# zzz5y/street_crafter

Hardware: AMD Instinct MI355X
Metric: frames/sec @1M Gaussians 1920x1280 + PSNR vs ref; 1/2/4/8 MI355X (higher is better)
Workload: dtype f32

## Files before the change

### include/street_crafter_amd.h

```cpp
#ifndef STREET_CRAFTER_AMD_H
#define STREET_CRAFTER_AMD_H

#include <stddef.h>
#include <stdint.h>

#ifdef __cplusplus
extern "C" {
#endif

typedef void* sc_stream_t;

#define SC_OK 0
#define SC_EINVAL (-1)
#define SC_EWORKSPACE (-2)
#define SC_EUNSUPPORTED (-3)

const char* sc_version(void);
const char* sc_error_string(int code);
const char* sc_target_arch(void);
int sc_wait_i64(const int64_t* addr, int64_t value, int64_t timeout_us);

int sc_projection_fwd(const float* means, const float* quats, const float* scales,
                      const float* viewmats, const float* Ks, int C, int N, int width, int height,
                      float eps2d, float near_plane, float far_plane, float radius_clip,
// ... 2 lines not shown

int sc_projection_bwd(const float* means, const float* quats, const float* scales,
                      const float* viewmats, const float* Ks, int C, int N, int width, int height,
                      float eps2d, const int32_t* radii, const float* conics,
                      const float* compensations ,
                      const float* v_means2d, const float* v_depths, const float* v_conics,
                      const float* v_compensations ,
                      float* v_means, float* v_quats, float* v_scales, sc_stream_t stream);

size_t sc_isect_workspace_bytes(int64_t CN);
int sc_isect_count(const float* means2d, const int32_t* radii, int C, int N,
                   int tile_size, int tile_width, int tile_height,
                   int32_t* tiles_per_gauss, int64_t* total_dev, void* workspace, size_t ws_bytes,
                   sc_stream_t stream);
int sc_isect_emit(const float* means2d, const int32_t* radii, const float* depths, int C, int N,
                  int tile_size, int tile_width, int tile_height,
                  const int32_t* tiles_per_gauss, int64_t n_isects,
                  int64_t* isect_ids, int32_t* flatten_ids, void* workspace, size_t ws_bytes,
                  sc_stream_t stream);

size_t sc_radix_sort_workspace_bytes(int64_t n);
int sc_radix_sort_pairs_u64_i32(uint64_t* keys, int32_t* vals, uint64_t* tmp_keys, int32_t* tmp_vals,
                                int64_t n, int end_bit, void* workspace, size_t ws_bytes,
                                sc_stream_t stream);

size_t sc_isect_bin_workspace_bytes(int64_t CN, int C, int tile_width, int tile_height, int64_t n_records);
int sc_isect_bin_count(const float* means2d, const int32_t* radii, const float* depths, int C, int N,
                       int tile_size, int tile_width, int tile_height,
                       int32_t* tiles_per_gauss, int32_t* isect_offsets, int64_t* meta_dev ,
                       int64_t* meta_mirror , int64_t seq,
                       void* workspace, size_t ws_bytes,
                       const int32_t* tile_work ,
                       const float* viewmats ,
                       int32_t* view_registry ,
                       int32_t* tile_order ,
                       sc_stream_t stream);
int sc_view_slots(void);
int sc_view_registry_words(void);
int sc_isect_bin_bucket_capacity(void);
int sc_isect_split_limits(int64_t* out );
int64_t sc_isect_split_seg_bound(int64_t n_records, int nsb);
int sc_isect_split_bins(const uint64_t* keys, int64_t n, uint64_t lo, uint64_t hi, int32_t* bins);
int sc_isect_split_plan(const uint32_t* bin_counts, int cap, int32_t* range_of_bin, int32_t* n_ranges);
int sc_isect_bin_sort(const float* means2d, const int32_t* radii, const float* depths, int C, int N,
                      int tile_size, int tile_width, int tile_height,
                      const int32_t* isect_offsets, const int64_t* meta_dev,
                      void* count_workspace ,
                      int64_t capacity, int64_t rec_capacity, int64_t super_capacity,
                      int64_t* isect_ids , int32_t* flatten_ids,
                      void* workspace, size_t ws_bytes, sc_stream_t stream);
int sc_isect_ids_rebuild(const int32_t* flatten_ids, const int32_t* isect_offsets, const float* depths,
                         int C, int N, int tile_width, int tile_height, int64_t n_isects,
                         int64_t* isect_ids, sc_stream_t stream);
int sc_isect_bin_reset_cursors(void* count_workspace, int64_t CN, int C, int tile_width, int tile_height,
                               sc_stream_t stream);

int sc_isect_offsets(const int64_t* isect_ids, int64_t n_isects, int C, int tile_width,
                     int tile_height, int32_t* offsets, sc_stream_t stream);

int sc_sh_fwd(int degree, const float* dirs, const float* coeffs, const uint8_t* masks,
              int64_t M, int K, float* colors, sc_stream_t stream);
int sc_sh_bwd(int degree, const float* dirs, const float* coeffs, const uint8_t* masks,
              int64_t M, int K, const float* v_colors, float* v_coeffs, float* v_dirs,
              sc_stream_t stream);

int sc_rasterize_fwd(const float* means2d, const float* conics, const float* colors,
                     const float* opacities, const float* backgrounds, const uint8_t* tile_masks,
                     int C, int N, int D, int width, int height, int tile_size,
                     int tile_width, int tile_height,
                     const int32_t* isect_offsets, const int32_t* flatten_ids, int64_t n_isects,
                     float* render_colors, float* render_alphas,
                     int32_t* last_ids ,
                     const int32_t* tile_order ,
                     int32_t* tile_work ,
                     sc_stream_t stream);
int sc_tile_order_len(int total_tiles);
int sc_rasterize_bwd(const float* means2d, const float* conics, const float* colors,
                     const float* opacities, const float* backgrounds, const uint8_t* tile_masks,
                     int C, int N, int D, int width, int height, int tile_size,
                     int tile_width, int tile_height,
                     const int32_t* isect_offsets, const int32_t* flatten_ids, int64_t n_isects,
                     const float* render_alphas, const int32_t* last_ids,
                     const float* v_render_colors, const float* v_render_alphas,
                     float* v_means2d_abs, float* v_means2d, float* v_conics, float* v_colors,
                     float* v_opacities, const int32_t* tile_order ,
                     sc_stream_t stream);

size_t sc_knn_workspace_bytes(int64_t n);
int sc_knn3_mean_dist2(const float* points, int64_t n, float* out, void* workspace,
                       size_t ws_bytes, sc_stream_t stream);

int sc_point_project(const float* points, const float* colors, const float* opacities , float occ,
                     const float* radius_in , int N, const double* viewmat, double fx,
                     double fy, double cx, double cy, double focal_r, int width, int height, double near_plane,
                     double far_plane, int radius_mode, double scale, float knn_scale_down, int32_t* radii,
                     float* means2d, float* depths, float* records, sc_stream_t stream);
int sc_point_rasterize_fwd(const float* records, int N, int width, int height, int tile_width, int tile_height,
                           const int32_t* isect_offsets, const int32_t* flatten_ids, int64_t n_isects, int max_hit,
                           const float* background , float* out_rgb, int64_t pix_stride,
                           int64_t ch_stride, float* out_alpha, int64_t alpha_stride,
                           float* out_depth , sc_stream_t stream);

size_t sc_loss_workspace_bytes(int batch, int channels, int height, int width);
int sc_loss_fwd(const float* img1, const float* img2, const uint8_t* mask , const int64_t* strides_host,
                int batch, int channels, int height, int width, int mask_batch, int mask_height, int mask_width,
                int window, float* ssim_out, float* l1_out, int64_t* kept_out ,
// ... 80 lines not shown
} sc_densify_job;
typedef struct {
    const float* src_param;
    const float* src_exp_avg;
    const float* src_exp_avg_sq;
    float* dst_param;
    float* dst_exp_avg;
    float* dst_exp_avg_sq;
    const float* child;
    const int32_t* src_row;
    const uint8_t* slot;
    int64_t n, n_out;
    int32_t width;
    int32_t reserved;
} sc_densify_group;
int sc_densify_scan_block(void);
int sc_densify_max_jobs(void);
int sc_densify_max_groups(void);
size_t sc_densify_plan_workspace_bytes(const sc_densify_job* jobs_host, int n_jobs);
int sc_densify_plan(const sc_densify_job* jobs_host, int n_jobs, void* workspace, size_t workspace_bytes,
                    sc_stream_t stream);
int sc_densify_apply(const sc_densify_group* groups_host, int n_groups, sc_stream_t stream);

int sc_camera_centers(const float* viewmats, int C, float* out, sc_stream_t stream);
int sc_projection_sh_fwd(const float* means, const float* quats, const float* scales,
                         const float* opacities, const float* sh_coeffs, const float* viewmats,
                         const float* Ks, const float* camera_centers, int C, int N, int K,
                         int sh_degree, int width, int height, float eps2d, float near_plane,
                         float far_plane, float radius_clip, int antialiased, int32_t* radii,
                         float* means2d, float* depths, float* conics, float* opacities_out,
                         float* colors4,
                         float* records ,
                         sc_stream_t stream);
int sc_projection_sh_bwd(const float* means, const float* quats, const float* scales,
                         const float* opacities, const float* sh_coeffs, const float* viewmats,
                         const float* Ks, const float* camera_centers, int C, int N, int K,
                         int sh_degree, int width, int height, float eps2d, int antialiased,
                         const int32_t* radii, const float* conics, const float* v_means2d,
                         const float* v_depths, const float* v_conics, const float* v_opacities_out,
                         const float* v_colors4, float* v_means, float* v_quats, float* v_scales,
                         float* v_opacities, float* v_sh, sc_stream_t stream);
int sc_rasterize_fwd_packed(const float* records, const float* backgrounds, const uint8_t* tile_masks,
                            int C, int N, int width, int height, int tile_width, int tile_height,
                            const int32_t* isect_offsets, const int32_t* flatten_ids, int64_t n_isects,
                            float* render_colors, float* render_alphas, const int32_t* tile_order,
                            int32_t* tile_work, int depth_normalise, sc_stream_t stream);
int sc_rasterize_fwd_planar(const float* means2d, const float* conics, const float* colors,
                            const float* opacities, const float* backgrounds, const uint8_t* tile_masks,
                            int C, int N, int D, int width, int height, int tile_size,
                            int tile_width, int tile_height,
                            const int32_t* isect_offsets, const int32_t* flatten_ids, int64_t n_isects,
                            float* render_colors, float* render_alphas,
                            const int32_t* tile_order, int32_t* tile_work, sc_stream_t stream);
int sc_records_unpack(const float* records, int64_t CN, float* conics, float* opacities, float* colors4,
                      sc_stream_t stream);
int sc_rasterize_fwd_ed(const float* means2d, const float* conics, const float* colors,
                        const float* opacities, const float* backgrounds, const uint8_t* tile_masks,
                        int C, int N, int D, int width, int height, int tile_size, int tile_width,
                        int tile_height, const int32_t* isect_offsets, const int32_t* flatten_ids,
                        int64_t n_isects, float* render_colors, float* render_alphas,
                        const int32_t* tile_order, int32_t* tile_work, sc_stream_t stream);

int sc_group_extents(const int32_t* isect_offsets, const int32_t* flatten_ids, int64_t n_isects,
                     const uint8_t* group_ids , int C, int N, int n_groups,
                     int tile_width, int tile_height, int32_t* group_end, sc_stream_t stream);
int sc_rasterize_fwd_groups(const float* means2d, const float* conics, const float* colors,
                            const float* opacities, const uint8_t* group_ids, const int32_t* group_end,
                            int C, int N, int D, int n_groups, int width, int height, int tile_size,
                            int tile_width, int tile_height,
                            const int32_t* isect_offsets, const int32_t* flatten_ids, int64_t n_isects,
                            float* render_colors, float* render_alphas,
                            float* group_colors, float* group_alphas, sc_stream_t stream);

int sc_rasterize_fwd_groups_ids(const float* means2d, const float* conics, const float* colors,
                                const float* opacities, const uint8_t* group_ids, const int32_t* group_end,
                                int C, int N, int D, int n_groups, int width, int height, int tile_size,
                                int tile_width, int tile_height,
                                const int32_t* isect_offsets, const int32_t* flatten_ids, int64_t n_isects,
                                float* render_colors, float* render_alphas,
                                float* group_colors, float* group_alphas, int32_t* last_pos, sc_stream_t stream);
int sc_rasterize_bwd_groups(const float* means2d, const float* conics, const float* colors,
                            const float* opacities, const uint8_t* group_ids, int C, int N, int D, int n_groups,
                            int width, int height, int tile_size, int tile_width, int tile_height,
                            const int32_t* isect_offsets, const int32_t* flatten_ids, int64_t n_isects,
                            const float* render_alphas, const float* group_alphas, const int32_t* last_pos,
                            const float* v_render_colors, const float* v_render_alphas,
                            const float* v_group_colors, const float* v_group_alphas,
                            float* v_means2d_abs, float* v_means2d, float* v_conics, float* v_colors,
                            float* v_opacities, sc_stream_t stream);

int sc_rasterize_fwd_layers(const float* means2d, const float* conics, const float* colors,
                            const float* opacities, int C, int N, int D, int n_front, int width, int height,
                            int tile_size, int tile_width, int tile_height,
                            const int32_t* isect_offsets, const int32_t* flatten_ids, int64_t n_isects,
                            int epilogue, int rounding, float* out0, float* out1, float* out2, float* out3,
                            uint8_t* out_u8, int32_t* layer_begin, sc_stream_t stream);

int sc_frame_composite_u8(const float* fg, int fg_stride, const float* acc, const float* sky, int sky_stride,
                          int64_t n_pixels, int rounding, uint8_t* out, sc_stream_t stream);
int sc_frame_composite_u8_strided(const float* fg, int64_t fg_pix_stride, int64_t fg_ch_stride, const float* acc,
                                  const float* sky, int64_t sky_pix_stride, int64_t sky_ch_stride, int64_t n_pixels,
                                  int rounding, uint8_t* out, sc_stream_t stream);

int sc_test_wave_transpose_sum16(const float* in, int n_waves, float* out, sc_stream_t stream);

int sc_test_tile_cull(const float* records, const int32_t* geometry, int n, int32_t* verdict, uint32_t* valid,
// ... 13 lines not shown
```

### street_crafter_amd/_ctypes_binding.py

```python
from __future__ import annotations

import ctypes

import torch

from . import _lib


def _p(t):
    return None if t is None else t.data_ptr()


def _ws(nbytes: int, device):
    return torch.empty(max(int(nbytes), 256), dtype=torch.uint8, device=device)


def projection_fwd(means, quats, scales, viewmats, Ks, width, height, eps2d, near_plane, far_plane, radius_clip,
                   calc_comp, stream):
    C, N = viewmats.shape[0], means.shape[0]
    dev = means.device
    radii = torch.empty((C, N), dtype=torch.int32, device=dev)
    means2d = torch.empty((C, N, 2), dtype=torch.float32, device=dev)
    depths = torch.empty((C, N), dtype=torch.float32, device=dev)
    conics = torch.empty((C, N, 3), dtype=torch.float32, device=dev)
    comps = torch.empty((C, N), dtype=torch.float32, device=dev) if calc_comp else None
    rc = _lib.load().sc_projection_fwd(_p(means), _p(quats), _p(scales), _p(viewmats), _p(Ks), C, N, int(width),
                                       int(height), float(eps2d), float(near_plane), float(far_plane),
                                       float(radius_clip), _p(radii), _p(means2d), _p(depths), _p(conics), _p(comps),
                                       stream)
    return rc, radii, means2d, depths, conics, comps


def projection_bwd(means, quats, scales, viewmats, Ks, width, height, eps2d, radii, conics, comps, v_means2d,
                   v_depths, v_conics, v_comps, stream):
    C, N = viewmats.shape[0], means.shape[0]
    v_means = torch.empty_like(means)
    v_quats = torch.empty_like(quats)
    v_scales = torch.empty_like(scales)
    rc = _lib.load().sc_projection_bwd(_p(means), _p(quats), _p(scales), _p(viewmats), _p(Ks), C, N, width, height,
                                       eps2d, _p(radii), _p(conics), _p(comps), _p(v_means2d), _p(v_depths),
                                       _p(v_conics), _p(v_comps), _p(v_means), _p(v_quats), _p(v_scales), stream)
    return rc, v_means, v_quats, v_scales


def isect_bin_count(means2d, radii, depths, tile_size, tile_width, tile_height, tile_work, viewmats, registry,
                    want_order, meta_host_ptr, seq, stream):
    lib = _lib.load()
    C, N = radii.shape
    dev = means2d.device
    tiles_per_gauss = torch.empty((C, N), dtype=torch.int32, device=dev)
    offsets = torch.empty((C, tile_height, tile_width), dtype=torch.int32, device=dev)
    meta_dev = torch.empty(4, dtype=torch.int64, device=dev)
    ws0 = _ws(lib.sc_isect_bin_workspace_bytes(C * N, C, tile_width, tile_height, -1), dev)
    order = (torch.empty(lib.sc_tile_order_len(C * tile_width * tile_height), dtype=torch.int32, device=dev)
             if want_order else None)
    rc = lib.sc_isect_bin_count(_p(means2d), _p(radii), _p(depths), C, N, int(tile_size), int(tile_width),
                                int(tile_height), _p(tiles_per_gauss), _p(offsets), _p(meta_dev), meta_host_ptr, seq,
                                _p(ws0), ws0.numel(), _p(tile_work) if want_order else None, _p(viewmats),
                                _p(registry), _p(order), stream)
    return rc, tiles_per_gauss, offsets, meta_dev, ws0, order


def isect_bin_sort(means2d, radii, depths, tile_size, tile_width, tile_height, offsets, meta_dev, ws0, capacity,
                   rec_capacity, super_capacity, want_ids, stream):
    lib = _lib.load()
    C, N = radii.shape
    dev = means2d.device
    ids = torch.empty(capacity, dtype=torch.int64, device=dev) if want_ids else None
    fids = torch.empty(capacity, dtype=torch.int32, device=dev)
    ws = _ws(lib.sc_isect_bin_workspace_bytes(C * N, C, tile_width, tile_height, rec_capacity), dev)
    rc = lib.sc_isect_bin_sort(_p(means2d), _p(radii), _p(depths), C, N, int(tile_size), int(tile_width),
                               int(tile_height), _p(offsets), _p(meta_dev), _p(ws0), capacity, rec_capacity,
                               super_capacity, _p(ids), _p(fids), _p(ws), ws.numel(), stream)
    return rc, ids, fids


def wait_i64(addr, value, timeout_us):
    return _lib.load().sc_wait_i64(addr, value, timeout_us)


def sh_fwd(degree, dirs, coeffs, masks, stream):
    M = dirs.numel() // 3
    K = coeffs.shape[-2]
    colors = torch.empty(dirs.shape, dtype=torch.float32, device=dirs.device)
    rc = _lib.load().sc_sh_fwd(int(degree), _p(dirs), _p(coeffs), _p(masks), M, K, _p(colors), stream)
    return rc, colors


def sh_bwd(degree, dirs, coeffs, masks, v_colors, need_dirs, stream):
    M = dirs.numel() // 3
    K = coeffs.shape[-2]
    v_coeffs = torch.empty_like(coeffs)
    v_dirs = torch.empty_like(dirs) if need_dirs else None
    rc = _lib.load().sc_sh_bwd(degree, _p(dirs), _p(coeffs), _p(masks), M, K, _p(v_colors), _p(v_coeffs), _p(v_dirs),
                               stream)
    return rc, v_coeffs, v_dirs


def rasterize_fwd(means2d, conics, colors, opacities, backgrounds, masks, width, height, tile_size, offsets,
                  flatten_ids, want_last, order, work, stream):
    C, N = opacities.shape
    D = colors.shape[-1]
    th, tw = offsets.shape[1], offsets.shape[2]
    dev = means2d.device
    render_colors = torch.empty((C, height, width, D), dtype=torch.float32, device=dev)
    render_alphas = torch.empty((C, height, width, 1), dtype=torch.float32, device=dev)
    last_ids = torch.empty((C, height, width), dtype=torch.int32, device=dev) if want_last else None
    rc = _lib.load().sc_rasterize_fwd(_p(means2d), _p(conics), _p(colors), _p(opacities), _p(backgrounds), _p(masks),
                                      C, N, D, int(width), int(height), int(tile_size), tw, th, _p(offsets),
                                      _p(flatten_ids), flatten_ids.numel(), _p(render_colors), _p(render_alphas),
                                      _p(last_ids), _p(order), _p(work), stream)
    return rc, render_colors, render_alphas, last_ids


def rasterize_fwd_planar(means2d, conics, colors, opacities, backgrounds, masks, width, height, tile_size, offsets,
                         flatten_ids, order, work, stream):
    C, N = opacities.shape
    D = colors.shape[-1]
    th, tw = offsets.shape[1], offsets.shape[2]
    dev = means2d.device
    planes = torch.empty((C, D, height, width), dtype=torch.float32, device=dev)
    render_alphas = torch.empty((C, height, width, 1), dtype=torch.float32, device=dev)
    rc = _lib.load().sc_rasterize_fwd_planar(_p(means2d), _p(conics), _p(colors), _p(opacities), _p(backgrounds),
                                             _p(masks), C, N, D, int(width), int(height), int(tile_size), tw, th,
                                             _p(offsets), _p(flatten_ids), flatten_ids.numel(), _p(planes),
                                             _p(render_alphas), _p(order), _p(work), stream)
    return rc, planes.permute(0, 2, 3, 1), render_alphas


def rasterize_fwd_groups(means2d, conics, colors, opacities, group_ids, n_groups, width, height, tile_size, offsets,
                         flatten_ids, stream):
    lib = _lib.load()
    C, N = opacities.shape
    D = colors.shape[-1]
    th, tw = offsets.shape[1], offsets.shape[2]
    G = max(int(n_groups), 0)
    dev = means2d.device
    render_colors = torch.empty((C, height, width, D), dtype=torch.float32, device=dev)
    render_alphas = torch.empty((C, height, width, 1), dtype=torch.float32, device=dev)
    group_colors = torch.empty((G, C, height, width, D), dtype=torch.float32, device=dev)
    group_alphas = torch.empty((G, C, height, width, 1), dtype=torch.float32, device=dev)
    group_end = torch.empty((C * th * tw, G), dtype=torch.int32, device=dev)
    rc = lib.sc_group_extents(_p(offsets), _p(flatten_ids), flatten_ids.numel(), _p(group_ids), C, N, int(n_groups), tw,
                              th, _p(group_end), stream)
    if rc == 0:
        rc = lib.sc_rasterize_fwd_groups(_p(means2d), _p(conics), _p(colors), _p(opacities), _p(group_ids),
                                         _p(group_end), C, N, D, int(n_groups), int(width), int(height),
                                         int(tile_size), tw, th, _p(offsets), _p(flatten_ids), flatten_ids.numel(),
                                         _p(render_colors), _p(render_alphas), _p(group_colors), _p(group_alphas),
                                         stream)
    return rc, render_colors, render_alphas, group_colors, group_alphas, group_end


def rasterize_fwd_layers(means2d, conics, colors, opacities, n_front, width, height, tile_size, offsets, flatten_ids,
                         epilogue, rounding, want_layer_begin, out, stream):
    C, N = opacities.shape
    D = colors.shape[-1]
    th, tw = offsets.shape[1], offsets.shape[2]
    dev = means2d.device

    def f32(*shape):
        return torch.empty(shape, dtype=torch.float32, device=dev)

    o0 = o1 = o2 = o3 = None
    if epilogue == 0:
        o0, o1, o2, o3 = f32(C, height, width, D), f32(C, height, width, 1), f32(C, height, width, 3), f32(C, height, width, 1)
    elif epilogue == 1:
        o0, o1 = f32(C, height, width, 3), f32(C, height, width, 1)
        o2 = f32(C, height, width, 1) if D == 4 else None
    elif epilogue == 2:
        if out is not None:
            if out.dtype != torch.uint8 or not out.is_cuda or not out.is_contiguous() or out.numel() != C * height * width * 3:
                raise RuntimeError("out must be a contiguous uint8 tensor of C*H*W*3 bytes on a HIP device")
            o0 = out
        else:
            o0 = torch.empty((C, height, width, 3), dtype=torch.uint8, device=dev)
    lb = torch.empty(C * th * tw, dtype=torch.int32, device=dev) if want_layer_begin else None
    u8_out = epilogue == 2
    rc = _lib.load().sc_rasterize_fwd_layers(_p(means2d), _p(conics), _p(colors), _p(opacities), C, N, D, int(n_front),
                                             int(width), int(height), int(tile_size), tw, th, _p(offsets),
# ... 296 lines not shown
```

### street_crafter_amd/_lib.py

```python
from __future__ import annotations

import ctypes as C
import os

_HERE = os.path.dirname(os.path.abspath(__file__))
LIB_PATH = os.path.join(_HERE, "lib", "libstreet_crafter_hip.so")
DIAG_LIB_PATH = os.path.join(_HERE, "lib", "libstreet_crafter_hip_diag.so")

_lib = None
_path = LIB_PATH
_lock = __import__("threading").Lock()


def use_diagnostic_build(tag: str = ""):
    global _path
    want = DIAG_LIB_PATH.replace("_diag.so", f"_diag_{tag}.so") if tag else DIAG_LIB_PATH
    if _lib is not None and _path != want:
        raise RuntimeError("use_diagnostic_build() must be called before the library is first loaded")
    if not os.path.exists(want):
        raise ImportError(f"diagnostic library not built ({want} missing): "
                          "python -m street_crafter_amd.build --diag")
    _path = want

c_f32p = C.c_void_p
# ... 16 lines not shown

class DensifyJob(C.Structure):
    _fields_ = [("n", C.c_int64), ("xyz", C.c_void_p), ("scaling", C.c_void_p), ("rotation", C.c_void_p),
                ("opacity", C.c_void_p), ("grad_accum", C.c_void_p), ("denom", C.c_void_p), ("max_radii", C.c_void_p),
                ("split_noise", C.c_void_p), ("box_noise", C.c_void_p), ("src_row", C.c_void_p), ("slot", C.c_void_p),
                ("child_xyz", C.c_void_p), ("child_scaling", C.c_void_p), ("counters", C.c_void_p),
                ("max_grad", C.c_float), ("dense_size", C.c_float), ("min_opacity", C.c_float), ("big_size", C.c_float),
                ("max_screen_size", C.c_float), ("region_a", C.c_float * 3), ("region_b", C.c_float * 3),
                ("grad_col", C.c_int32), ("prune_big", C.c_int32), ("region", C.c_int32)]


class DensifyGroup(C.Structure):
    _fields_ = [("src_param", C.c_void_p), ("src_exp_avg", C.c_void_p), ("src_exp_avg_sq", C.c_void_p),
                ("dst_param", C.c_void_p), ("dst_exp_avg", C.c_void_p), ("dst_exp_avg_sq", C.c_void_p),
                ("child", C.c_void_p), ("src_row", C.c_void_p), ("slot", C.c_void_p), ("n", C.c_int64),
                ("n_out", C.c_int64), ("width", C.c_int32), ("reserved", C.c_int32)]


SIGNATURES = {
    "sc_version": (C.c_char_p, []),
    "sc_error_string": (C.c_char_p, [C.c_int]),
    "sc_wait_i64": (C.c_int, [C.c_void_p, C.c_int64, C.c_int64]),
    "sc_target_arch": (C.c_char_p, []),
    "sc_projection_fwd": (C.c_int, [c_f32p, c_f32p, c_f32p, c_f32p, c_f32p, C.c_int, C.c_int, C.c_int,
                                    C.c_int, C.c_float, C.c_float, C.c_float, C.c_float, c_i32p, c_f32p,
                                    c_f32p, c_f32p, c_f32p, c_stream]),
    "sc_projection_bwd": (C.c_int, [c_f32p, c_f32p, c_f32p, c_f32p, c_f32p, C.c_int, C.c_int, C.c_int,
                                    C.c_int, C.c_float, c_i32p, c_f32p, c_f32p, c_f32p, c_f32p, c_f32p,
                                    c_f32p, c_f32p, c_f32p, c_f32p, c_stream]),
    "sc_isect_workspace_bytes": (C.c_size_t, [C.c_int64]),
    "sc_isect_count": (C.c_int, [c_f32p, c_i32p, C.c_int, C.c_int, C.c_int, C.c_int, C.c_int, c_i32p,
                                 c_i64p, C.c_void_p, C.c_size_t, c_stream]),
    "sc_isect_emit": (C.c_int, [c_f32p, c_i32p, c_f32p, C.c_int, C.c_int, C.c_int, C.c_int, C.c_int,
                                c_i32p, C.c_int64, c_i64p, c_i32p, C.c_void_p, C.c_size_t, c_stream]),
    "sc_radix_sort_workspace_bytes": (C.c_size_t, [C.c_int64]),
    "sc_radix_sort_pairs_u64_i32": (C.c_int, [c_u64p, c_i32p, c_u64p, c_i32p, C.c_int64, C.c_int,
                                              C.c_void_p, C.c_size_t, c_stream]),
    "sc_isect_bin_workspace_bytes": (C.c_size_t, [C.c_int64, C.c_int, C.c_int, C.c_int, C.c_int64]),
    "sc_isect_bin_count": (C.c_int, [c_f32p, c_i32p, c_f32p, C.c_int, C.c_int, C.c_int, C.c_int, C.c_int, c_i32p,
                                     c_i32p, c_i64p, c_i64p, C.c_int64, C.c_void_p, C.c_size_t, c_i32p, c_f32p, c_i32p,
                                     c_i32p, c_stream]),
    "sc_view_slots": (C.c_int, []),
    "sc_view_registry_words": (C.c_int, []),
    "sc_isect_bin_bucket_capacity": (C.c_int, []),
    "sc_isect_split_limits": (C.c_int, [c_i64p]),
    "sc_isect_split_seg_bound": (C.c_int64, [C.c_int64, C.c_int]),
    "sc_isect_split_bins": (C.c_int, [c_u64p, C.c_int64, C.c_uint64, C.c_uint64, c_i32p]),
    "sc_isect_split_plan": (C.c_int, [C.c_void_p, C.c_int, c_i32p, c_i32p]),
    "sc_isect_bin_sort": (C.c_int, [c_f32p, c_i32p, c_f32p, C.c_int, C.c_int, C.c_int, C.c_int, C.c_int,
                                    c_i32p, c_i64p, C.c_void_p, C.c_int64, C.c_int64, C.c_int64, c_i64p,
                                    c_i32p, C.c_void_p, C.c_size_t, c_stream]),
    "sc_isect_ids_rebuild": (C.c_int, [c_i32p, c_i32p, c_f32p, C.c_int, C.c_int, C.c_int, C.c_int, C.c_int64, c_i64p,
                                       c_stream]),
    "sc_isect_bin_reset_cursors": (C.c_int, [C.c_void_p, C.c_int64, C.c_int, C.c_int, C.c_int, c_stream]),
    "sc_isect_offsets": (C.c_int, [c_i64p, C.c_int64, C.c_int, C.c_int, C.c_int, c_i32p, c_stream]),
    "sc_sh_fwd": (C.c_int, [C.c_int, c_f32p, c_f32p, c_u8p, C.c_int64, C.c_int, c_f32p, c_stream]),
    "sc_sh_bwd": (C.c_int, [C.c_int, c_f32p, c_f32p, c_u8p, C.c_int64, C.c_int, c_f32p, c_f32p, c_f32p,
                            c_stream]),
    "sc_rasterize_fwd": (C.c_int, [c_f32p, c_f32p, c_f32p, c_f32p, c_f32p, c_u8p, C.c_int, C.c_int, C.c_int,
                                   C.c_int, C.c_int, C.c_int, C.c_int, C.c_int, c_i32p, c_i32p, C.c_int64,
                                   c_f32p, c_f32p, c_i32p, c_i32p, c_i32p, c_stream]),
    "sc_rasterize_fwd_ed": (C.c_int, [c_f32p, c_f32p, c_f32p, c_f32p, c_f32p, c_u8p, C.c_int, C.c_int, C.c_int,
                                      C.c_int, C.c_int, C.c_int, C.c_int, C.c_int, c_i32p, c_i32p, C.c_int64,
                                      c_f32p, c_f32p, c_i32p, c_i32p, c_stream]),
    "sc_rasterize_fwd_planar": (C.c_int, [c_f32p, c_f32p, c_f32p, c_f32p, c_f32p, c_u8p, C.c_int, C.c_int, C.c_int,
                                          C.c_int, C.c_int, C.c_int, C.c_int, C.c_int, c_i32p, c_i32p, C.c_int64,
                                          c_f32p, c_f32p, c_i32p, c_i32p, c_stream]),
    "sc_group_extents": (C.c_int, [c_i32p, c_i32p, C.c_int64, c_u8p, C.c_int, C.c_int, C.c_int, C.c_int, C.c_int,
                                   c_i32p, c_stream]),
    "sc_rasterize_fwd_groups": (C.c_int, [c_f32p, c_f32p, c_f32p, c_f32p, c_u8p, c_i32p, C.c_int, C.c_int, C.c_int,
                                          C.c_int, C.c_int, C.c_int, C.c_int, C.c_int, C.c_int, c_i32p, c_i32p,
                                          C.c_int64, c_f32p, c_f32p, c_f32p, c_f32p, c_stream]),
    "sc_rasterize_fwd_groups_ids": (C.c_int, [c_f32p, c_f32p, c_f32p, c_f32p, c_u8p, c_i32p, C.c_int, C.c_int, C.c_int,
                                              C.c_int, C.c_int, C.c_int, C.c_int, C.c_int, C.c_int, c_i32p, c_i32p,
                                              C.c_int64, c_f32p, c_f32p, c_f32p, c_f32p, c_i32p, c_stream]),
    "sc_rasterize_bwd_groups": (C.c_int, [c_f32p, c_f32p, c_f32p, c_f32p, c_u8p, C.c_int, C.c_int, C.c_int, C.c_int,
                                          C.c_int, C.c_int, C.c_int, C.c_int, C.c_int, c_i32p, c_i32p, C.c_int64,
                                          c_f32p, c_f32p, c_i32p, c_f32p, c_f32p, c_f32p, c_f32p, c_f32p, c_f32p,
                                          c_f32p, c_f32p, c_f32p, c_stream]),
    "sc_camera_centers": (C.c_int, [c_f32p, C.c_int, c_f32p, c_stream]),
    "sc_projection_sh_fwd": (C.c_int, [c_f32p, c_f32p, c_f32p, c_f32p, c_f32p, c_f32p, c_f32p, c_f32p,
                                       C.c_int, C.c_int, C.c_int, C.c_int, C.c_int, C.c_int, C.c_float,
                                       C.c_float, C.c_float, C.c_float, C.c_int, c_i32p, c_f32p, c_f32p,
                                       c_f32p, c_f32p, c_f32p, c_f32p, c_stream]),
    "sc_projection_sh_bwd": (C.c_int, [c_f32p, c_f32p, c_f32p, c_f32p, c_f32p, c_f32p, c_f32p, c_f32p,
                                       C.c_int, C.c_int, C.c_int, C.c_int, C.c_int, C.c_int, C.c_float, C.c_int,
                                       c_i32p, c_f32p, c_f32p, c_f32p, c_f32p, c_f32p, c_f32p, c_f32p, c_f32p,
                                       c_f32p, c_f32p, c_f32p, c_stream]),
    "sc_rasterize_fwd_packed": (C.c_int, [c_f32p, c_f32p, c_u8p, C.c_int, C.c_int, C.c_int, C.c_int, C.c_int, C.c_int,
                                          c_i32p, c_i32p, C.c_int64, c_f32p, c_f32p, c_i32p, c_i32p, C.c_int, c_stream]),
    "sc_records_unpack": (C.c_int, [c_f32p, C.c_int64, c_f32p, c_f32p, c_f32p, c_stream]),
    "sc_tile_order_len": (C.c_int, [C.c_int]),
    "sc_rasterize_bwd": (C.c_int, [c_f32p, c_f32p, c_f32p, c_f32p, c_f32p, c_u8p, C.c_int, C.c_int, C.c_int,
                                   C.c_int, C.c_int, C.c_int, C.c_int, C.c_int, c_i32p, c_i32p, C.c_int64,
                                   c_f32p, c_i32p, c_f32p, c_f32p, c_f32p, c_f32p, c_f32p, c_f32p, c_f32p,
                                   c_i32p, c_stream]),
    "sc_knn_workspace_bytes": (C.c_size_t, [C.c_int64]),
    "sc_knn3_mean_dist2": (C.c_int, [c_f32p, C.c_int64, c_f32p, C.c_void_p, C.c_size_t, c_stream]),
    "sc_rasterize_fwd_layers": (C.c_int, [c_f32p, c_f32p, c_f32p, c_f32p, C.c_int, C.c_int, C.c_int, C.c_int, C.c_int,
                                          C.c_int, C.c_int, C.c_int, C.c_int, c_i32p, c_i32p, C.c_int64, C.c_int, C.c_int,
                                          c_f32p, c_f32p, c_f32p, c_f32p, c_u8p, c_i32p, c_stream]),
    "sc_frame_composite_u8": (C.c_int, [c_f32p, C.c_int, c_f32p, c_f32p, C.c_int, C.c_int64, C.c_int, c_u8p,
                                        c_stream]),
    "sc_frame_composite_u8_strided": (C.c_int, [c_f32p, C.c_int64, C.c_int64, c_f32p, c_f32p, C.c_int64, C.c_int64, C.c_int64,
                                                C.c_int, c_u8p, c_stream]),
    "sc_point_project": (C.c_int, [c_f32p, c_f32p, c_f32p, C.c_float, c_f32p, C.c_int, c_f32p, C.c_double, C.c_double,
# ... 156 lines not shown
```

### street_crafter_amd/csrc/binding.cpp

```cpp
#include <torch/extension.h>

#include <algorithm>
#include <cstdint>
#include <tuple>
#include <vector>

#include "../../include/street_crafter_amd.h"

#ifndef SC_ABI_HASH
#define SC_ABI_HASH "unhashed"
#endif

namespace {

using at::Tensor;
using OptT = c10::optional<Tensor>;

inline sc_stream_t S(int64_t s) { return reinterpret_cast<sc_stream_t>(static_cast<uintptr_t>(s)); }

inline void req(const Tensor& t, at::ScalarType dt, const char* name) {
    TORCH_CHECK(t.is_cuda(), name, " must live on a HIP device (got ", t.device(), "); street_crafter_amd has no CPU path");
    TORCH_CHECK(t.scalar_type() == dt, name, " must be ", dt, ", got ", t.scalar_type());
    TORCH_CHECK(t.is_contiguous(), name, " must be contiguous");
}
// ... 48 lines not shown
    return {rc, v_means, v_quats, v_scales};
}
py::tuple projection_bwd(const Tensor& means, const Tensor& quats, const Tensor& scales, const Tensor& viewmats,
                         const Tensor& Ks, int64_t width, int64_t height, double eps2d, const Tensor& radii,
                         const Tensor& conics, const OptT& comps, const Tensor& v_means2d, const Tensor& v_depths,
                         const Tensor& v_conics, const OptT& v_comps, int64_t stream) {
    ProjBwdT o = projection_bwd_c(means, quats, scales, viewmats, Ks, width, height, eps2d, radii, conics, comps, v_means2d,
                                  v_depths, v_conics, v_comps, stream);
    return py::make_tuple(o.rc, o.v_means, o.v_quats, o.v_scales);
}

py::tuple isect_bin_count(const Tensor& means2d, const Tensor& radii, const Tensor& depths, int64_t tile_size,
                          int64_t tile_width, int64_t tile_height, const OptT& tile_work, const OptT& viewmats,
                          const OptT& registry, bool want_order, int64_t meta_host_ptr, int64_t seq, int64_t stream) {
    req(means2d, at::kFloat, "means2d"); req(radii, at::kInt, "radii"); req(depths, at::kFloat, "depths");
    const int64_t C = radii.size(0), N = radii.size(1);
    Tensor tpg = at::empty({C, N}, i32(means2d));
    Tensor offsets = at::empty({C, tile_height, tile_width}, i32(means2d));
    Tensor meta_dev = at::empty({4}, means2d.options().dtype(at::kLong));
    size_t wsb = sc_isect_bin_workspace_bytes(C * N, (int)C, (int)tile_width, (int)tile_height, -1);
    if (wsb < 256) wsb = 256;
    Tensor ws0 = at::empty({(int64_t)wsb}, u8(means2d));
    OptT order;
    if (want_order) order = at::empty({(int64_t)sc_tile_order_len((int)(C * tile_width * tile_height))}, i32(means2d));
    const int rc = sc_isect_bin_count(
        fp(means2d), ip(radii), fp(depths), (int)C, (int)N, (int)tile_size, (int)tile_width, (int)tile_height,
        static_cast<int32_t*>(tpg.data_ptr()), static_cast<int32_t*>(offsets.data_ptr()),
        static_cast<int64_t*>(meta_dev.data_ptr()), reinterpret_cast<int64_t*>(static_cast<uintptr_t>(meta_host_ptr)), seq,
        ws0.data_ptr(), wsb, (want_order && tile_work) ? ip(*tile_work) : nullptr, viewmats ? fp(*viewmats) : nullptr,
        registry ? static_cast<int32_t*>(registry->data_ptr()) : nullptr,
        order ? static_cast<int32_t*>(order->data_ptr()) : nullptr, S(stream));
    return py::make_tuple(rc, tpg, offsets, meta_dev, ws0, order);
}

py::tuple isect_bin_sort(const Tensor& means2d, const Tensor& radii, const Tensor& depths, int64_t tile_size,
                         int64_t tile_width, int64_t tile_height, const Tensor& offsets, const Tensor& meta_dev,
                         const Tensor& ws0, int64_t capacity, int64_t rec_capacity, int64_t super_capacity, bool want_ids,
                         int64_t stream) {
    const int64_t C = radii.size(0), N = radii.size(1);
    OptT ids;
    if (want_ids) ids = at::empty({capacity}, means2d.options().dtype(at::kLong));
    Tensor fids = at::empty({capacity}, i32(means2d));
    size_t wsb = sc_isect_bin_workspace_bytes(C * N, (int)C, (int)tile_width, (int)tile_height, rec_capacity);
    if (wsb < 256) wsb = 256;
    Tensor ws = at::empty({(int64_t)wsb}, u8(means2d));
    const int rc = sc_isect_bin_sort(fp(means2d), ip(radii), fp(depths), (int)C, (int)N, (int)tile_size, (int)tile_width,
                                     (int)tile_height, ip(offsets), static_cast<const int64_t*>(meta_dev.data_ptr()),
                                     ws0.data_ptr(), capacity, rec_capacity, super_capacity,
                                     ids ? static_cast<int64_t*>(ids->data_ptr()) : nullptr,
                                     static_cast<int32_t*>(fids.data_ptr()), ws.data_ptr(), wsb, S(stream));
    return py::make_tuple(rc, ids, fids);
}

int wait_i64(int64_t addr, int64_t value, int64_t timeout_us) {
    py::gil_scoped_release nogil;
    return sc_wait_i64(reinterpret_cast<const int64_t*>(static_cast<uintptr_t>(addr)), value, timeout_us);
}

struct ShFwdT { int rc; Tensor colors; };
ShFwdT sh_fwd_c(int64_t degree, const Tensor& dirs, const Tensor& coeffs, const OptT& masks, int64_t stream) {
    req(dirs, at::kFloat, "dirs"); req(coeffs, at::kFloat, "coeffs");
    if (masks) req(*masks, at::kByte, "masks");
    const int64_t M = dirs.numel() / 3, K = coeffs.size(-2);
    Tensor colors = at::empty(dirs.sizes(), f32(dirs));
    const int rc = sc_sh_fwd((int)degree, fp(dirs), fp(coeffs), masks ? static_cast<const uint8_t*>(masks->data_ptr()) : nullptr,
                             M, (int)K, fpw(colors), S(stream));
    return {rc, colors};
}
py::tuple sh_fwd(int64_t degree, const Tensor& dirs, const Tensor& coeffs, const OptT& masks, int64_t stream) {
    ShFwdT o = sh_fwd_c(degree, dirs, coeffs, masks, stream);
    return py::make_tuple(o.rc, o.colors);
}

struct ShBwdT { int rc; Tensor v_coeffs; OptT v_dirs; };
ShBwdT sh_bwd_c(int64_t degree, const Tensor& dirs, const Tensor& coeffs, const OptT& masks, const Tensor& v_colors,
                bool need_dirs, int64_t stream) {
    req(v_colors, at::kFloat, "v_colors");
    const int64_t M = dirs.numel() / 3, K = coeffs.size(-2);
    Tensor v_coeffs = at::empty_like(coeffs);
    OptT v_dirs;
    if (need_dirs) v_dirs = at::empty_like(dirs);
    const int rc = sc_sh_bwd((int)degree, fp(dirs), fp(coeffs), masks ? static_cast<const uint8_t*>(masks->data_ptr()) : nullptr,
                             M, (int)K, fp(v_colors), fpw(v_coeffs), v_dirs ? fpw(*v_dirs) : nullptr, S(stream));
    return {rc, v_coeffs, v_dirs};
}
py::tuple sh_bwd(int64_t degree, const Tensor& dirs, const Tensor& coeffs, const OptT& masks, const Tensor& v_colors,
                 bool need_dirs, int64_t stream) {
    ShBwdT o = sh_bwd_c(degree, dirs, coeffs, masks, v_colors, need_dirs, stream);
    return py::make_tuple(o.rc, o.v_coeffs, o.v_dirs);
}

struct RasterFwdT { int rc; Tensor colors, alphas; OptT last; };
RasterFwdT rasterize_fwd_c(const Tensor& means2d, const Tensor& conics, const Tensor& colors, const Tensor& opacities,
                           const OptT& backgrounds, const OptT& masks, int64_t width, int64_t height, int64_t tile_size,
                           const Tensor& offsets, const Tensor& flatten_ids, bool want_last, const OptT& order,
                           const OptT& work, int64_t stream) {
    req(means2d, at::kFloat, "means2d"); req(conics, at::kFloat, "conics"); req(colors, at::kFloat, "colors");
    req(opacities, at::kFloat, "opacities"); req(offsets, at::kInt, "isect_offsets"); req(flatten_ids, at::kInt, "flatten_ids");
    const int64_t C = opacities.size(0), N = opacities.size(1), D = colors.size(-1);
    const int64_t th = offsets.size(1), tw = offsets.size(2);
    Tensor rc_ = at::empty({C, height, width, D}, f32(means2d));
    Tensor ra = at::empty({C, height, width, 1}, f32(means2d));
    OptT last;
    if (want_last) last = at::empty({C, height, width}, i32(means2d));
    const int rc = sc_rasterize_fwd(fp(means2d), fp(conics), fp(colors), fp(opacities), fpo(backgrounds),
                                    masks ? static_cast<const uint8_t*>(masks->data_ptr()) : nullptr, (int)C, (int)N, (int)D,
                                    (int)width, (int)height, (int)tile_size, (int)tw, (int)th, ip(offsets), ip(flatten_ids),
                                    flatten_ids.numel(), fpw(rc_), fpw(ra),
                                    last ? static_cast<int32_t*>(last->data_ptr()) : nullptr,
                                    order ? ip(*order) : nullptr, work ? static_cast<int32_t*>(work->data_ptr()) : nullptr,
                                    S(stream));
    return {rc, rc_, ra, last};
}
py::tuple rasterize_fwd_planar(const Tensor& means2d, const Tensor& conics, const Tensor& colors, const Tensor& opacities,
                               const OptT& backgrounds, const OptT& masks, int64_t width, int64_t height, int64_t tile_size,
                               const Tensor& offsets, const Tensor& flatten_ids, const OptT& order, const OptT& work,
                               int64_t stream) {
    req(means2d, at::kFloat, "means2d"); req(conics, at::kFloat, "conics"); req(colors, at::kFloat, "colors");
    req(opacities, at::kFloat, "opacities"); req(offsets, at::kInt, "isect_offsets"); req(flatten_ids, at::kInt, "flatten_ids");
    const int64_t C = opacities.size(0), N = opacities.size(1), D = colors.size(-1);
    const int64_t th = offsets.size(1), tw = offsets.size(2);
    Tensor planes = at::empty({C, D, height, width}, f32(means2d));
    Tensor ra = at::empty({C, height, width, 1}, f32(means2d));
    const int rc = sc_rasterize_fwd_planar(fp(means2d), fp(conics), fp(colors), fp(opacities), fpo(backgrounds),
                                           masks ? static_cast<const uint8_t*>(masks->data_ptr()) : nullptr, (int)C, (int)N,
                                           (int)D, (int)width, (int)height, (int)tile_size, (int)tw, (int)th, ip(offsets),
                                           ip(flatten_ids), flatten_ids.numel(), fpw(planes), fpw(ra),
                                           order ? ip(*order) : nullptr,
                                           work ? static_cast<int32_t*>(work->data_ptr()) : nullptr, S(stream));
    return py::make_tuple(rc, planes.permute({0, 2, 3, 1}), ra);
}
py::tuple rasterize_fwd_groups(const Tensor& means2d, const Tensor& conics, const Tensor& colors, const Tensor& opacities,
                               const Tensor& group_ids, int64_t n_groups, int64_t width, int64_t height, int64_t tile_size,
                               const Tensor& offsets, const Tensor& flatten_ids, int64_t stream) {
    req(means2d, at::kFloat, "means2d"); req(conics, at::kFloat, "conics"); req(colors, at::kFloat, "colors");
    req(opacities, at::kFloat, "opacities"); req(offsets, at::kInt, "isect_offsets"); req(flatten_ids, at::kInt, "flatten_ids");
    req(group_ids, at::kByte, "group_ids");
    const int64_t C = opacities.size(0), N = opacities.size(1), D = colors.size(-1);
    const int64_t th = offsets.size(1), tw = offsets.size(2), G = std::max<int64_t>(n_groups, 0);
    Tensor rc_ = at::empty({C, height, width, D}, f32(means2d));
    Tensor ra = at::empty({C, height, width, 1}, f32(means2d));
    Tensor gc = at::empty({G, C, height, width, D}, f32(means2d));
    Tensor ga = at::empty({G, C, height, width, 1}, f32(means2d));
    Tensor ge = at::empty({C * th * tw, G}, i32(means2d));
    const uint8_t* gid = static_cast<const uint8_t*>(group_ids.data_ptr());
    int rc = sc_group_extents(ip(offsets), ip(flatten_ids), flatten_ids.numel(), gid, (int)C, (int)N, (int)n_groups, (int)tw,
                              (int)th, static_cast<int32_t*>(ge.data_ptr()), S(stream));
    if (rc == 0)
        rc = sc_rasterize_fwd_groups(fp(means2d), fp(conics), fp(colors), fp(opacities), gid, ip(ge), (int)C, (int)N, (int)D,
                                     (int)n_groups, (int)width, (int)height, (int)tile_size, (int)tw, (int)th, ip(offsets),
                                     ip(flatten_ids), flatten_ids.numel(), fpw(rc_), fpw(ra), fpw(gc), fpw(ga), S(stream));
    return py::make_tuple(rc, rc_, ra, gc, ga, ge);
}
py::tuple rasterize_fwd_layers(const Tensor& means2d, const Tensor& conics, const Tensor& colors, const Tensor& opacities,
                               int64_t n_front, int64_t width, int64_t height, int64_t tile_size, const Tensor& offsets,
                               const Tensor& flatten_ids, int64_t epilogue, int64_t rounding, bool want_layer_begin,
                               const OptT& out, int64_t stream) {
    req(means2d, at::kFloat, "means2d"); req(conics, at::kFloat, "conics"); req(colors, at::kFloat, "colors");
    req(opacities, at::kFloat, "opacities"); req(offsets, at::kInt, "isect_offsets"); req(flatten_ids, at::kInt, "flatten_ids");
    const int64_t C = opacities.size(0), N = opacities.size(1), D = colors.size(-1);
    const int64_t th = offsets.size(1), tw = offsets.size(2);
    OptT o0, o1, o2, o3, lb;
    if (epilogue == 0) {
        o0 = at::empty({C, height, width, D}, f32(means2d));
        o1 = at::empty({C, height, width, 1}, f32(means2d));
        o2 = at::empty({C, height, width, 3}, f32(means2d));
        o3 = at::empty({C, height, width, 1}, f32(means2d));
    } else if (epilogue == 1) {
        o0 = at::empty({C, height, width, 3}, f32(means2d));
        o1 = at::empty({C, height, width, 1}, f32(means2d));
        if (D == 4) o2 = at::empty({C, height, width, 1}, f32(means2d));
    } else if (epilogue == 2) {
        if (out) {
            req(*out, at::kByte, "out");
            TORCH_CHECK(out->numel() == C * height * width * 3, "out must hold C*H*W*3 bytes");
            o0 = *out;
        } else {
            o0 = at::empty({C, height, width, 3}, u8(means2d));
        }
    }
    if (want_layer_begin) lb = at::empty({C * th * tw}, i32(means2d));
    auto w = [](const OptT& t) { return t ? static_cast<float*>(t->data_ptr()) : nullptr; };
    const bool u8_out = epilogue == 2;
// ... 590 lines not shown
py::tuple densify_apply(const std::vector<Tensor>& src_param, const std::vector<OptT>& src_exp_avg,
                        const std::vector<OptT>& src_exp_avg_sq, const std::vector<OptT>& child,
                        const std::vector<Tensor>& src_row, const std::vector<Tensor>& slot, const std::vector<int64_t>& n,
                        const std::vector<int64_t>& n_out, const std::vector<int64_t>& width, int64_t stream) {
    const size_t G = src_param.size();
    TORCH_CHECK(src_exp_avg.size() == G && src_exp_avg_sq.size() == G && child.size() == G && src_row.size() == G &&
                slot.size() == G && n.size() == G && n_out.size() == G && width.size() == G,
                "densify_apply: lists of different length");
    std::vector<Tensor> dst_param(G);
    std::vector<OptT> dst_m(G), dst_v(G);
    std::vector<sc_densify_group> groups(G);
    for (size_t k = 0; k < G; ++k) {
        req(src_param[k], at::kFloat, "param"); req(src_row[k], at::kInt, "src_row"); req(slot[k], at::kByte, "slot");
        TORCH_CHECK(n[k] >= 0 && n_out[k] >= 0 && width[k] >= 0 && width[k] <= INT32_MAX &&
                    src_param[k].numel() == n[k] * width[k] && src_row[k].numel() >= n_out[k] && slot[k].numel() >= n_out[k],
                    "densify_apply: group ", k, ": sizes do not match");
        TORCH_CHECK(src_exp_avg[k].has_value() == src_exp_avg_sq[k].has_value(), "densify_apply: group ", k, ": one moment");
        sc_densify_group& g = groups[k];
        g = sc_densify_group{};
        dst_param[k] = at::empty({n_out[k], width[k]}, f32(src_param[k]));
        g.src_param = fp(src_param[k]); g.dst_param = fpw(dst_param[k]);
        if (src_exp_avg[k]) {
            req(*src_exp_avg[k], at::kFloat, "exp_avg"); req(*src_exp_avg_sq[k], at::kFloat, "exp_avg_sq");
            TORCH_CHECK(src_exp_avg[k]->numel() == n[k] * width[k] && src_exp_avg_sq[k]->numel() == n[k] * width[k],
                        "densify_apply: group ", k, ": moments differ in size from the parameter");
            dst_m[k] = at::empty({n_out[k], width[k]}, f32(src_param[k]));
            dst_v[k] = at::empty({n_out[k], width[k]}, f32(src_param[k]));
            if (n_out[k] * width[k] > 0) {
                g.src_exp_avg = fp(*src_exp_avg[k]); g.src_exp_avg_sq = fp(*src_exp_avg_sq[k]);
                g.dst_exp_avg = fpw(*dst_m[k]); g.dst_exp_avg_sq = fpw(*dst_v[k]);
            }
        }
        if (child[k]) {
            req(*child[k], at::kFloat, "child");
            TORCH_CHECK(child[k]->numel() == 2 * n[k] * width[k], "densify_apply: group ", k, ": child rows are not [2,n,width]");
            g.child = fp(*child[k]);
        }
        g.src_row = ip(src_row[k]); g.slot = static_cast<const uint8_t*>(slot[k].data_ptr());
        g.n = n[k]; g.n_out = n_out[k]; g.width = (int32_t)width[k];
    }
    const int rc = sc_densify_apply(groups.data(), (int)G, S(stream));
    return py::make_tuple(rc, dst_param, dst_m, dst_v);
}

}

PYBIND11_MODULE(TORCH_EXTENSION_NAME, m) {
    m.doc() = "street_crafter_amd: compiled Python <-> C-ABI binding layer (allocation + call per operator)";
    m.def("abi_version", []() { return std::string("street_crafter_amd 0.4.0 (gfx950) abi:" SC_ABI_HASH); });
    m.def("projection_fwd", &projection_fwd);
    m.def("projection_bwd", &projection_bwd);
    m.def("isect_bin_count", &isect_bin_count);
    m.def("isect_bin_sort", &isect_bin_sort);
    m.def("wait_i64", &wait_i64);
    m.def("sh_fwd", &sh_fwd);
    m.def("sh_bwd", &sh_bwd);
    m.def("rasterize_fwd", &rasterize_fwd);
    m.def("rasterize_fwd_planar", &rasterize_fwd_planar);
    m.def("rasterize_fwd_groups", &rasterize_fwd_groups);
    m.def("rasterize_fwd_layers", &rasterize_fwd_layers);
    m.def("rasterize_fwd_groups_ids", &rasterize_fwd_groups_ids);
    m.def("rasterize_bwd_groups", &rasterize_bwd_groups);
    m.def("rasterize_bwd", &rasterize_bwd);
    m.def("projection_autograd", &projection_autograd);
    m.def("sh_autograd", &sh_autograd);
    m.def("rasterize_autograd", &rasterize_autograd);
    m.def("projection_sh_fwd", &projection_sh_fwd);
    m.def("projection_sh_bwd", &projection_sh_bwd);
    m.def("rasterize_fwd_packed", &rasterize_fwd_packed);
    m.def("frame_composite_u8", &frame_composite_u8);
    m.def("frame_composite_u8_strided", &frame_composite_u8_strided);
    m.def("loss_fwd", &loss_fwd);
    m.def("loss_bwd", &loss_bwd);
    m.def("depth_trim_fwd", &depth_trim_fwd);
    m.def("depth_trim_bwd", &depth_trim_bwd);
    m.def("acc_reg_fwd", &acc_reg_fwd);
    m.def("acc_reg_bwd", &acc_reg_bwd);
    m.def("cubemap_fwd", &cubemap_fwd);
    m.def("cubemap_bwd", &cubemap_bwd);
    m.def("adam_step", &adam_step);
    m.def("densify_stats", &densify_stats);
    m.def("densify_plan", &densify_plan);
    m.def("densify_apply", &densify_apply);
}
```

### street_crafter_amd/csrc/isect_bin.hip

```cpp
#include "sc_common.h"

#pragma clang fp contract(off)

#include "isect_split_plan.h"

namespace {

constexpr int BIN_THREADS = 1024;
constexpr int BIN_GPT = 4;
constexpr int BIN_GPB = BIN_THREADS * BIN_GPT;
constexpr int CNT_GPT = 8;
constexpr int BIN_MAX_TILES = 36864;
constexpr int BIN_BIG = 32;
constexpr unsigned ID_MASK = 0x0fffffffu;
constexpr unsigned long long KEY_MASK = 0xffffffff0fffffffull;

struct Rect { int x0, x1, y0, y1; };

struct Geo {
    int tile_width, tile_height, T;
    int ss;
    int stw, sth, ST;
    int N;
};
// ... 618 lines not shown
        unsigned long long carry = 0;
        for (int b0 = 0; b0 < cnt; b0 += 64) {
            const int i = b0 + lane;
            const unsigned long long v = (i < cnt) ? table[i] : 0ull;
            const unsigned long long incl = (unsigned long long)sc_wave_incl_scan64((long long)v);
            if (i < cnt) table[i] = carry + incl - v;
            carry += (unsigned long long)__shfl((long long)incl, 63, 64);
        }
        if (totals && lane < 4) totals[lane] = (unsigned)((carry >> (16 * lane)) & 0xffffu);
    }
    __syncthreads();
    long long hi_key[4];
    int tbase[4], tend[4];
    bool tok[4];
#pragma unroll
    for (int k = 0; k < 4; ++k) {
        const int tx = (sx << g.ss) + (k & 1), ty = (sy << g.ss) + (k >> 1);
        tok[k] = (k < ntile) && tx < g.tile_width && ty < g.tile_height;
        const int tile = ty * g.tile_width + tx;
        const int tflat = cam * g.T + tile;
        tbase[k] = tok[k] ? offsets[tflat] + tb[k] : 0;
        tend[k] = tok[k] ? ((tflat + 1 < n_tiles_total) ? offsets[tflat + 1] : (int)n_isects) : 0;
        hi_key[k] = ((long long)cam << (32 + tile_bits)) | ((long long)tile << 32);
    }
    if (SC_DIAG_BIT(dbg, 1)) return;
    for (int r = 0; r < rounds; ++r) {
        const int i = r * THREADS + t;
        const unsigned long long key = (i < n) ? S[order ? order[i] : i] : 0ull;
        const unsigned m = (i < n) ? (unsigned)((key >> 28) & 0xfu) : 0u;
        const unsigned long long base = table[r * WAVES + wave];
#pragma unroll
        for (int k = 0; k < 4; ++k) {
            const unsigned long long bal = __ballot((m >> k) & 1u);
            if (((m >> k) & 1u) && tok[k]) {
                const int pos = tbase[k] + (int)((base >> (16 * k)) & 0xffffu) + __popcll(bal & sc_lanemask_lt());
                if (pos < tend[k]) {
                    if (isect_ids && !SC_DIAG_BIT(dbg, 16)) isect_ids[pos] = hi_key[k] | (long long)(key >> 32);
                    flatten_ids[pos] = (int32_t)((unsigned)key & ID_MASK);
                }
            }
        }
    }
}

__host__ __device__ inline size_t sort_lds_bytes(int cap, int threads = SS_THREADS) {
    const size_t table = (size_t)((cap + threads - 1) / threads + 1) * (threads / 64) * 8 + 64;
    return (size_t)cap * 10 + (size_t)((cap + 4) & ~1) * 4 + (size_t)threads * 4 + table + 16;
}

template <int THREADS, int RPT>
__device__ __forceinline__ void sort_segment(
    const uint2* __restrict__ recs, int n, int sb, const int* tb, int cap, const Geo& g,
    const int32_t* __restrict__ offsets, int n_tbuckets, int64_t n_isects, int tile_bits,
    unsigned char* smem, int64_t* __restrict__ isect_ids, int32_t* __restrict__ flatten_ids, unsigned* totals_out
    SC_DIAG_PARAM(dbg)) {
    constexpr int WAVES = THREADS / 64, NC = THREADS;
    unsigned long long* B = reinterpret_cast<unsigned long long*>(smem);
    unsigned short* order = reinterpret_cast<unsigned short*>(B + cap);
    unsigned* boff = reinterpret_cast<unsigned*>(order + cap);
    unsigned* coarse = boff + ((cap + 4) & ~1);
    unsigned long long* table = reinterpret_cast<unsigned long long*>(coarse + NC);
    unsigned* totals = reinterpret_cast<unsigned*>(reinterpret_cast<unsigned char*>(table) +
                                                   (size_t)((cap + THREADS - 1) / THREADS + 1) * WAVES * 8 + 64);
    __shared__ unsigned long long red_lo[WAVES], red_hi[WAVES];
    __shared__ unsigned red_sum[WAVES];
    const int t = threadIdx.x, lane = t & 63, wave = t >> 6;

    uint2 rec[RPT];
#pragma unroll
    for (int k = 0; k < RPT; ++k) {
        const int i = t + k * THREADS;
        rec[k] = (i < n) ? recs[i] : make_uint2(0u, 0u);
    }
    for (int i = t; i <= n; i += THREADS) boff[i] = 0;
    coarse[t] = 0u;
    unsigned long long lo = ~0ull, hi = 0ull;
#pragma unroll
    for (int k = 0; k < RPT; ++k) {
        if (t + k * THREADS < n) {
            const unsigned long long K = rec_key60(rec[k]);
            lo = K < lo ? K : lo;
            hi = K > hi ? K : hi;
        }
    }
#pragma unroll
    for (int o = 32; o >= 1; o >>= 1) {
        const unsigned long long l2 = (unsigned long long)__shfl_xor((long long)lo, o, 64);
        const unsigned long long h2 = (unsigned long long)__shfl_xor((long long)hi, o, 64);
        lo = l2 < lo ? l2 : lo;
        hi = h2 > hi ? h2 : hi;
    }
    if (lane == 0) { red_lo[wave] = lo; red_hi[wave] = hi; }
    __syncthreads();
    lo = red_lo[0]; hi = red_hi[0];
#pragma unroll
    for (int w = 1; w < WAVES; ++w) {
        lo = red_lo[w] < lo ? red_lo[w] : lo;
        hi = red_hi[w] > hi ? red_hi[w] : hi;
    }
    if (SC_DIAG_BIT(dbg, 4)) return;
    const double s1 = (double)NC / ((double)(hi - lo) + 1.0);
    auto level1 = [&](unsigned long long K, float& frac) -> int {
        const double p = (double)(K - lo) * s1;
        int c = (int)p;
        c = c < NC - 1 ? c : NC - 1;
        frac = (float)(p - (double)c);
        return c;
    };
// ... 36 lines not shown
    }
    __syncthreads();
    {
        const int per = ((n + THREADS - 1) / THREADS) | 1;
        const int beg = min(t * per, n), end = min(beg + per, n);
        unsigned sum = 0;
        for (int i = beg; i < end; ++i) sum += boff[i];
        const unsigned incl = (unsigned)sc_wave_incl_scan((int)sum);
        __syncthreads();
        if (lane == 63) red_sum[wave] = incl;
        __syncthreads();
        unsigned run = incl - sum;
#pragma unroll
        for (int w = 0; w < WAVES; ++w) if (w < wave) run += red_sum[w];
        for (int i = beg; i < end; ++i) {
            const unsigned c = boff[i];
            boff[i] = run;
            run += c;
        }
    }
    __syncthreads();
    if (SC_DIAG_BIT(dbg, 32)) return;
#pragma unroll
    for (int k = 0; k < RPT; ++k) {
        if (t + k * THREADS < n) {
            const uint2 r = rec[k];
            const int f = fj[k];
            const unsigned slot = atomicAdd(&boff[f], 1u);
            B[slot] = ((unsigned long long)r.x << 32) | r.y;
            order[slot] = (unsigned short)f;
        }
    }
    __syncthreads();
    if (SC_DIAG_BIT(dbg, 2)) return;
    unsigned short bj[RPT];
#pragma unroll
    for (int k = 0; k < RPT; ++k) {
        const int p = t + k * THREADS;
        bj[k] = p < n ? order[p] : (unsigned short)0;
    }
    __syncthreads();
#pragma unroll
    for (int k = 0; k < RPT; ++k) {
        const int p = t + k * THREADS;
        if (p >= n) break;
        const unsigned long long kk = B[p] & KEY_MASK;
        const int j = bj[k];
        const unsigned beg = j > 0 ? boff[j - 1] : 0u, end = boff[j];
        unsigned r = beg;
        for (unsigned q = beg; q < end; ++q) r += ((B[q] & KEY_MASK) < kk) ? 1u : 0u;
        order[r] = (unsigned short)p;
    }
    __syncthreads();
    emit_tiles<THREADS>(B, order, n, sb, g, offsets, n_tbuckets, n_isects, tile_bits, tb, table, isect_ids,
                           flatten_ids, totals SC_DIAG_ARG(dbg));
    if (totals_out) {
        __syncthreads();
        if (t < 4) totals_out[t] = totals[t];
    }
}

__device__ __forceinline__ void sort_heavy_segment(
    const uint2* __restrict__ src, uint2* __restrict__ dst, int n, int sb, const int* tb_in, int cap, const Geo& g,
    const int32_t* __restrict__ offsets, int n_tbuckets, int64_t n_isects, int tile_bits, unsigned char* smem,
    int64_t* __restrict__ isect_ids, int32_t* __restrict__ flatten_ids) {
    unsigned long long* B = reinterpret_cast<unsigned long long*>(smem);
    unsigned long long* table = reinterpret_cast<unsigned long long*>(smem + (size_t)cap * 8);
    __shared__ unsigned tot[4];
    __shared__ int tbr[4];
    const int t = threadIdx.x;
    for (int i = t; i < n; i += SS_THREADS) {
        const uint2 r = src[i];
        const unsigned long long K = rec_key60(r);
        int rank = 0;
        for (int j = 0; j < n; ++j) rank += rec_key60(src[j]) < K ? 1 : 0;
        dst[rank] = r;
    }
    if (t < 4) tbr[t] = tb_in[t];
    __threadfence();
    __syncthreads();
    for (int c0 = 0; c0 < n; c0 += cap) {
        const int m = min(cap, n - c0);
        for (int i = t; i < m; i += SS_THREADS) {
            const unsigned long long v = __hip_atomic_load(reinterpret_cast<const unsigned long long*>(dst + c0 + i),
                                                           __ATOMIC_RELAXED, __HIP_MEMORY_SCOPE_AGENT);
            B[i] = (v << 32) | (v >> 32);
        }
        __syncthreads();
        int tbl[4] = {tbr[0], tbr[1], tbr[2], tbr[3]};
        emit_tiles<SS_THREADS>(B, nullptr, m, sb, g, offsets, n_tbuckets, n_isects, tile_bits, tbl, table, isect_ids,
                               flatten_ids, tot SC_DIAG_ARG(0));
        __syncthreads();
        if (t < 4) tbr[t] += (int)tot[t];
        __syncthreads();
    }
}

template <int THREADS, int RPT>
__global__ __launch_bounds__(THREADS, 6) void super_sort_kernel(
    const uint2* __restrict__ records, uint2* __restrict__ records_rw, const uint2* __restrict__ temp,
    const Segment* __restrict__ segs, const unsigned* __restrict__ n_segs, int seg_bound,
    const int32_t* __restrict__ soffsets, int n_sbuckets, int n_tbuckets,
    Geo g, const int32_t* __restrict__ offsets, const int64_t* __restrict__ meta, int64_t capacity,
    int64_t rec_capacity, int64_t super_capacity, int tile_bits, int cap,
    int64_t* __restrict__ isect_ids, int32_t* __restrict__ flatten_ids SC_DIAG_PARAM(dbg)) {
    extern __shared__ __align__(16) unsigned char smem[];
    if (meta[0] > capacity || meta[2] > rec_capacity || meta[3] > super_capacity) return;
    __shared__ int tb_s[4];
    if (THREADS == SS_THREADS && (int)blockIdx.x < seg_bound) {
        if (blockIdx.x >= *n_segs) return;
        const Segment* sg = segs + blockIdx.x;
        if (threadIdx.x < 4) tb_s[threadIdx.x] = sg->tb[threadIdx.x];
        const int start = sg->start, sn = sg->n, ssb = sg->sb;
        __syncthreads();
        if (sg->heavy)
            sort_heavy_segment(temp + start, records_rw + start, sn, ssb, tb_s, cap, g, offsets, n_tbuckets,
                               meta[0], tile_bits, smem, isect_ids, flatten_ids);
        else
            sort_segment<SS_THREADS, SS_RPT>(temp + start, sn, ssb, tb_s, cap, g, offsets, n_tbuckets, meta[0], tile_bits,
                                             smem, isect_ids, flatten_ids, nullptr SC_DIAG_ARG(dbg));
        return;
    }
    const int sb = (int)blockIdx.x - seg_bound;
    const int s = soffsets[sb];
    const int e = (sb + 1 < n_sbuckets) ? soffsets[sb + 1] : (int)meta[2];
    const int n = e - s;
    if (n <= 0 || n > cap) return;
    if (threadIdx.x < 4) tb_s[threadIdx.x] = 0;
    __syncthreads();
    sort_segment<THREADS, RPT>(records + s, n, sb, tb_s, cap, g, offsets, n_tbuckets, meta[0], tile_bits, smem, isect_ids,
                               flatten_ids, nullptr SC_DIAG_ARG(dbg));
}

__global__ __launch_bounds__(256) void isect_ids_rebuild_kernel(
    const int32_t* __restrict__ flatten_ids, const int32_t* __restrict__ offsets, const float* __restrict__ depths,
    int n_tiles_total, int tiles_per_cam, int tile_bits, int64_t CN, int64_t n_isects, int64_t* __restrict__ isect_ids) {
    const int tflat = blockIdx.x;
    const int cam = tflat / tiles_per_cam, tile = tflat - cam * tiles_per_cam;
    int s = offsets[tflat];
    int e = (tflat + 1 < n_tiles_total) ? offsets[tflat + 1] : (int)n_isects;
    s = min(max(s, 0), (int)n_isects);
    e = min(max(e, s), (int)n_isects);
    const long long hi = ((long long)cam << (32 + tile_bits)) | ((long long)tile << 32);
    for (int k = s + (int)threadIdx.x; k < e; k += 256) {
        const int g = flatten_ids[k];
        const unsigned d = ((unsigned)g < (unsigned)CN) ? __float_as_uint(depths[g]) : 0u;
        isect_ids[k] = hi | (long long)d;
    }
}

constexpr int BS_THREADS = 1024;
constexpr int BS_NB = SP_BINS;
constexpr int BS_MAX_RANGES = 256;
static_assert(BS_NB == BS_THREADS, "thread t owns bin t");
static_assert(2 * (BIG_MAX_SUPER / (SS_MAX_CAP + 1)) + 1 <= BS_MAX_RANGES, "range tables: isect_split_plan.h, THE BOUND");
constexpr int BS_UNROLL = 8;

template <typename F>
__device__ __forceinline__ void for_records(const uint2* __restrict__ src, int n, F&& f) {
    for (int i0 = threadIdx.x; i0 < n; i0 += BS_THREADS * BS_UNROLL) {
        uint2 v[BS_UNROLL];
#pragma unroll
        for (int u = 0; u < BS_UNROLL; ++u) {
            const int i = i0 + u * BS_THREADS;
            v[u] = i < n ? src[i] : make_uint2(0u, 0u);
        }
#pragma unroll
        for (int u = 0; u < BS_UNROLL; ++u)
            if (i0 + u * BS_THREADS < n) f(v[u]);
    }
}

__global__ __launch_bounds__(BS_THREADS, 8) void big_split_kernel(
    const uint2* __restrict__ records, uint2* __restrict__ temp, Segment* __restrict__ segs,
    unsigned* __restrict__ n_segs, int seg_bound, const int32_t* __restrict__ soffsets, int n_sbuckets,
    const int64_t* __restrict__ meta, int64_t capacity, int64_t rec_capacity, int64_t super_capacity, int cap
    SC_DIAG_PARAM(dbg)) {
    if (meta[0] > capacity || meta[2] > rec_capacity || meta[3] > super_capacity) return;
    constexpr int REP = 8;
    __shared__ unsigned hist[BS_NB * REP];
    constexpr int TREP = 4;
    __shared__ unsigned rcnt[BS_MAX_RANGES], rtile[BS_MAX_RANGES][4][TREP], rstart[BS_MAX_RANGES], rcur[BS_MAX_RANGES];
    __shared__ unsigned long long red_lo[BS_THREADS / 64], red_hi[BS_THREADS / 64];
    __shared__ unsigned wtot[BS_THREADS / 64], wheavy[BS_THREADS / 64];
// ... 322 lines not shown
        else SC_LAUNCH_COUNT(true, 1, ldsb);
    } else {
        if (gpt == 8) SC_LAUNCH_COUNT(false, 8, 0);
        else if (gpt == 4) SC_LAUNCH_COUNT(false, 4, 0);
        else if (gpt == 2) SC_LAUNCH_COUNT(false, 2, 0);
        else SC_LAUNCH_COUNT(false, 1, 0);
    }
#undef SC_LAUNCH_COUNT
    SC_LAUNCH_CHECK();
    ScanJobs jobs;
    jobs.j[0] = ScanJob{(const int*)dgrid_t, C, tile_width, tile_height, isect_offsets, meta_dev, 1};
    jobs.j[1] = ScanJob{(const int*)dgrid_s, C, L.g.stw, L.g.sth, soffsets, meta_dev + 2, 1};
    jobs.j[2] = jobs.j[1];
    unsigned* scans_done = (unsigned*)(ws + L.scans_done);
    size_t center_lds = (size_t)L.nsb * 12 > (size_t)L.nt_cells * 4 ? (size_t)L.nsb * 12 : (size_t)L.nt_cells * 4;
    const size_t n_fwd_items = (size_t)L.ntb + L.ntb / 8 + 8;
    const size_t order_lds_staged = 4096 + ((size_t)L.ntb + 2) * 2 + n_fwd_items * 2 + 16;
    const int staged = tile_order && order_lds_staged <= 150 * 1024;
    const size_t order_lds = staged ? order_lds_staged : 4096 + ((size_t)L.ntb + 2) * 2 + 16;
    if (tile_order && center_lds < order_lds) center_lds = order_lds;
    hipLaunchKernelGGL(center_scatter_kernel, dim3(grid + 3), dim3(BIN_THREADS), center_lds, s,
                       (const int32_t*)tiles_per_gauss, means2d, radii, CN, L.g, (float)tile_size, L.nsb,
                       depths, (const unsigned*)chist, ccursor, sorted, cmeta, jobs, scans_done, meta_dev,
                       meta_mirror, seq, (const unsigned*)whint, (const unsigned*)wstat, tile_order, L.ntb, staged,
                       g_sc_raster_split, g_sc_raster_bwd_split ? 0 : 1 SC_DIAG_ARG(g_sc_debug[1] >> 16));
    SC_LAUNCH_CHECK();
    return SC_OK;
}

extern "C" int sc_isect_bin_reset_cursors(void* count_workspace, int64_t CN, int C, int tile_width, int tile_height,
                                          sc_stream_t stream) {
    if (!count_workspace || C <= 0 || tile_width <= 0 || tile_height <= 0) return SC_EINVAL;
    if ((int64_t)C * tile_width * tile_height > BIN_MAX_TILES) return SC_EUNSUPPORTED;
    const BinLayout L = bin_layout(CN, C, 1, tile_width, tile_height);
    SC_HIP(hipMemsetAsync((unsigned char*)count_workspace + L.rcursor, 0, L.scans_done - L.rcursor, sc_s(stream)));
    return SC_OK;
}

extern "C" int sc_isect_ids_rebuild(const int32_t* flatten_ids, const int32_t* isect_offsets, const float* depths,
                                    int C, int N, int tile_width, int tile_height, int64_t n_isects,
                                    int64_t* isect_ids, sc_stream_t stream) {
    if (C < 0 || N < 0 || tile_width <= 0 || tile_height <= 0 || n_isects < 0 || n_isects > 0x7fffffffLL) return SC_EINVAL;
    if (C == 0 || n_isects == 0) return SC_OK;
    if (!flatten_ids || !isect_offsets || !depths || !isect_ids) return SC_EINVAL;
    const int64_t nb = (int64_t)C * tile_width * tile_height;
    if (nb > 0x7fffffffLL) return SC_EINVAL;
    hipLaunchKernelGGL(isect_ids_rebuild_kernel, dim3((unsigned)nb), dim3(256), 0, sc_s(stream), flatten_ids, isect_offsets,
                       depths, (int)nb, tile_width * tile_height, sc_bits_for((int64_t)tile_width * tile_height),
                       (int64_t)C * N, n_isects, isect_ids);
    SC_LAUNCH_CHECK();
    return SC_OK;
}

extern "C" int sc_isect_bin_sort(const float* means2d, const int32_t* radii, const float* depths, int C,
                                 int N, int tile_size, int tile_width, int tile_height,
                                 const int32_t* isect_offsets, const int64_t* meta_dev,
                                 void* count_workspace, int64_t capacity, int64_t rec_capacity,
                                 int64_t super_capacity, int64_t* isect_ids, int32_t* flatten_ids,
                                 void* workspace, size_t ws_bytes, sc_stream_t stream) {
    if (C < 0 || N < 0 || tile_size <= 0 || tile_width <= 0 || tile_height <= 0 || capacity < 0 ||
        rec_capacity < 0 || super_capacity < 0)
        return SC_EINVAL;
    const int64_t CN = (int64_t)C * N;
    const int64_t nb64 = (int64_t)C * tile_width * tile_height;
    if (nb64 > BIN_MAX_TILES || CN >= (1LL << 28) || capacity > 0x7fffffffLL) return SC_EUNSUPPORTED;
    if (capacity == 0 || CN == 0) return SC_OK;
    if (super_capacity > BIG_MAX_SUPER) return SC_EUNSUPPORTED;
    const bool big = super_capacity > SS_MAX_CAP;
    int cap = big ? SS_MAX_CAP : (int)((super_capacity + 255) / 256 * 256);
    if (cap < 256) cap = 256;
    if (!means2d || !radii || !depths || !isect_offsets || !meta_dev || !count_workspace || !flatten_ids ||
        !workspace)
        return SC_EINVAL;
    if (ws_bytes < sc_isect_bin_workspace_bytes(CN, C, tile_width, tile_height, rec_capacity)) return SC_EWORKSPACE;
    hipStream_t s = sc_s(stream);
    const BinLayout L = bin_layout(CN, C, N, tile_width, tile_height);
    unsigned char* cws = (unsigned char*)count_workspace;
    const int32_t* soffsets = (const int32_t*)(cws + L.soffsets);
    const int64_t* cmeta = (const int64_t*)(cws + L.cmeta);
    const uint4* sorted = (const uint4*)(cws + L.sorted);
    unsigned* cursor = (unsigned*)(cws + L.rcursor);
    unsigned* n_segs = (unsigned*)(cws + L.nseg);
    const size_t rec_bytes = sc_align_up((size_t)rec_capacity * 8, 256);
    uint2* records = (uint2*)workspace;
    uint2* temp = (uint2*)((unsigned char*)workspace + rec_bytes);
    Segment* segs = (Segment*)((unsigned char*)workspace + 2 * rec_bytes);
    const int seg_bound = big ? (int)seg_bound_for(rec_capacity, L.nsb) : 0;
    const bool few_huge = CN <= 262144 && (rec_capacity > 32 * CN || CN < 32768);
    if (!few_huge)
        hipLaunchKernelGGL((bin_scatter_flat_kernel<FLAT_THREADS, 64>), dim3((unsigned)((CN + FLAT_THREADS - 1) / FLAT_THREADS)),
                           dim3(FLAT_THREADS), (size_t)L.nsb * 8 + 16 + (FLAT_THREADS / 64) * sizeof(FlatTab), s, sorted, cmeta,
                           L.g, L.nsb, soffsets, meta_dev, capacity, rec_capacity, super_capacity, cursor, records
                           SC_DIAG_ARG(g_sc_debug[0]));
    else {
        constexpr int gpb = FLAT_THREADS_SMALL / 64 * 16;
        hipLaunchKernelGGL((bin_scatter_flat_kernel<FLAT_THREADS_SMALL, 16>), dim3((unsigned)((CN + gpb - 1) / gpb)),
                           dim3(FLAT_THREADS_SMALL), (size_t)L.nsb * 8 + 16 + (FLAT_THREADS_SMALL / 64) * sizeof(FlatTab), s,
                           sorted, cmeta, L.g, L.nsb, soffsets, meta_dev, capacity, rec_capacity, super_capacity, cursor,
                           records SC_DIAG_ARG(g_sc_debug[0]));
    }
    SC_LAUNCH_CHECK();
    const int tile_bits = sc_bits_for(L.g.T);
    SC_HIP(bin_attrs_once());
    if (big) {
        const int bgrid = L.nsb;
        hipLaunchKernelGGL(big_split_kernel, dim3(bgrid), dim3(BS_THREADS), 0, s, (const uint2*)records, temp, segs,
                           n_segs, seg_bound, soffsets, L.nsb, meta_dev, capacity, rec_capacity, super_capacity, cap SC_DIAG_ARG(g_sc_debug[3]));
        SC_LAUNCH_CHECK();
    }
#define SC_LAUNCH_SORT(THREADSP, RPTP, GRID, LDSB, SEGB)                                                                      \
    hipLaunchKernelGGL((super_sort_kernel<THREADSP, RPTP>), dim3(GRID), dim3(THREADSP), LDSB, s,                              \
                       (const uint2*)records, records, (const uint2*)temp, (const Segment*)segs, (const unsigned*)n_segs, SEGB, \
                       soffsets, L.nsb, L.ntb, L.g, isect_offsets, meta_dev, capacity, rec_capacity, super_capacity, tile_bits,  \
                       cap, isect_ids, flatten_ids SC_DIAG_ARG(g_sc_debug[2]))
    if (!big && cap <= SS_SMALL_CAP)
        SC_LAUNCH_SORT(SS_SMALL_THREADS, SS_SMALL_RPT, (unsigned)L.nsb, sort_lds_bytes(cap, SS_SMALL_THREADS), 0);
    else
        SC_LAUNCH_SORT(SS_THREADS, SS_RPT, (unsigned)(seg_bound + L.nsb), sort_lds_bytes(cap), seg_bound);
#undef SC_LAUNCH_SORT
    SC_LAUNCH_CHECK();
    return SC_OK;
}
```

### street_crafter_amd/csrc/raster_fwd.hip

```cpp
#include "raster_walk.h"

int g_sc_raster_fwd_variant = 3;


namespace {

template <int CDIM>
__global__ void raster_fwd_ref_kernel(
    const float* __restrict__ means2d, const float* __restrict__ conics,
    const float* __restrict__ colors, const float* __restrict__ opacities,
    const float* __restrict__ backgrounds, const uint8_t* __restrict__ tile_masks, int N, int D,
    int width, int height, int tile_size, int tile_width, int tile_height,
    const int32_t* __restrict__ isect_offsets, const int32_t* __restrict__ flatten_ids, int n_isects,
    float* __restrict__ render_colors, float* __restrict__ render_alphas,
    int32_t* __restrict__ last_ids) {
    extern __shared__ __align__(16) unsigned char smem[];
    const int B = blockDim.x * blockDim.y;
    int* id_s = reinterpret_cast<int*>(smem);
    float4* xyoa_s = reinterpret_cast<float4*>(smem + (size_t)B * 16);
    float2* bc_s = reinterpret_cast<float2*>(smem + (size_t)B * 32);

    const int cam = blockIdx.z;
    const int tile_id = blockIdx.y * tile_width + blockIdx.x;
    const int tflat = cam * tile_width * tile_height + tile_id;
// ... 63 lines not shown
            for (int d = 0; d < ND; ++d)
                if (CDIM > 0 || d < D) pix_out[d] = __fmaf_rn(c[d], vis, pix_out[d]);
            cur_idx = batch_start + t;
            T = next_T;
        }
    }
    if (inside) {
        render_alphas[pix] = 1.0f - T;
#pragma unroll
        for (int d = 0; d < ND; ++d)
            if (CDIM > 0 || d < D)
                render_colors[pix * D + d] = backgrounds ? pix_out[d] + T * backgrounds[cam * D + d] : pix_out[d];
        if (last_ids) last_ids[pix] = cur_idx;
    }
}

#ifdef SC_DIAG
constexpr int SC_PHASE_ROWS = 65536;
__device__ unsigned long long g_sc_phase_cycles[SC_PHASE_ROWS][10];
__global__ void phase_sum_kernel(unsigned long long* out8, int reset) {
    __shared__ unsigned long long acc[10];
    if (threadIdx.x < 10) acc[threadIdx.x] = 0;
    __syncthreads();
    for (int r = threadIdx.x; r < SC_PHASE_ROWS; r += blockDim.x)
        for (int k = 0; k < 10; ++k) {
            const unsigned long long v = g_sc_phase_cycles[r][k];
            if (v) atomicAdd(&acc[k], v);
            if (reset) g_sc_phase_cycles[r][k] = 0;
        }
    __syncthreads();
    if (threadIdx.x < 10) out8[threadIdx.x] = acc[threadIdx.x];
}
extern "C" int sc_diag_phase_cycles(unsigned long long* out8, int reset) {
    unsigned long long* d = nullptr;
    hipError_t e = hipMalloc(&d, 80);
    if (e != hipSuccess) return (int)e;
    hipLaunchKernelGGL(phase_sum_kernel, dim3(1), dim3(1024), 0, 0, d, reset);
    e = hipDeviceSynchronize();
    if (e == hipSuccess && out8) e = hipMemcpy(out8, d, 80, hipMemcpyDeviceToHost);
    hipFree(d);
    return (int)e;
}
#endif

template <int CDIM, bool TRACK, int NSUB, bool PACKED = false, bool ED = false, bool PLANAR = false>
__device__ __forceinline__ void raster_item(
    const float* __restrict__ means2d, const float* __restrict__ conics,
    const float* __restrict__ colors, const float* __restrict__ opacities,
    const float* __restrict__ backgrounds, const uint8_t* __restrict__ tile_masks, int N,
    int width, int height, int tile_width, int tile_height, int total_tiles,
    const int32_t* __restrict__ isect_offsets, const int32_t* __restrict__ flatten_ids, int n_isects,
    float* __restrict__ render_colors, float* __restrict__ render_alphas,
    int32_t* __restrict__ last_ids, int tflat, int sub,
    float4* xyoa_s, float4* bck_s, float4* col_s, int32_t* __restrict__ tile_work SC_DIAG_PARAM(dbg)) {
    constexpr int B = SC_WALK_B;
    using Pixels = ScLanePixels<NSUB>;
    constexpr int NP = Pixels::NP, PPL = Pixels::PPL;

    const ScTileId tile = sc_tile_id(tflat, tile_width, tile_height);
    const int cam = tile.cam;
    const int lane = threadIdx.x;
    const Pixels px(tile, sub, lane, width, height);
    const bool (&inside)[PPL] = px.inside;
    const int64_t pix0 = px.pix0;

    const int64_t plane = (int64_t)height * width;
    const int64_t ppix0 = (int64_t)cam * CDIM * plane + (int64_t)px.py_i * width + px.px0_i;
    if (tile_masks && !tile_masks[tflat]) {
#pragma unroll
        for (int k = 0; k < PPL; ++k) {
            if (inside[k]) {
#pragma unroll
                for (int d = 0; d < CDIM; ++d)
                    render_colors[PLANAR ? ppix0 + d * plane + k : (pix0 + k) * CDIM + d] = backgrounds ? backgrounds[cam * CDIM + d] : 0.f;
                render_alphas[pix0 + k] = 0.f;
                if (last_ids) last_ids[pix0 + k] = 0;
            }
        }
        if (tile_work && lane == 0) tile_work[tflat] = 0;
        return;
    }
    const bool prof = SC_DIAG_BIT(dbg, 4);
    const unsigned long long pc_begin = SC_DIAG_CLOCK(prof), pr_begin = SC_DIAG_REALTIME(prof);
    unsigned long long pc_stage = 0, pc_issue = 0, pc_blend = 0, pc_first = 0, pc_batches = 0, pc_splats = 0;
    int range_start, range_end;
    sc_tile_range(isect_offsets, tflat, total_tiles, n_isects, range_start, range_end);
    const int num_batches = (range_end - range_start + B - 1) / B;
    int walked = 0;
    const ScRect rect = px.rect(tile, sub, width, height);

    const float INF = __builtin_huge_valf();
    sc_f2 pxp[NP], T2[NP];
    int cur[2 * NP];
    float acc[2 * NP][CDIM];
#pragma unroll
    for (int p = 0; p < NP; ++p) {
        pxp[p] = px.x_pair(p, px.px0_i, INF);
        T2[p] = sc_f2{1.f, 1.f};
    }
#pragma unroll
    for (int k = 0; k < 2 * NP; ++k) {
        cur[k] = 0;
#pragma unroll
        for (int d = 0; d < CDIM; ++d) acc[k][d] = 0.f;
    }
    auto all_done = [&]() -> bool { return sc_all_marked_x(pxp); };

    const ScSplatArrays in = {means2d, conics, colors, opacities};
    ScStage<CDIM, PACKED> st;
    st.clear();
    st.load(st.id_at(flatten_ids, range_start + lane, range_end, N), in);
    st.g_next = st.id_at(flatten_ids, range_start + B + lane, range_end, N);

    for (int b = 0; b < num_batches; ++b) {
        if (all_done()) break;
        const int batch_start = range_start + B * b;
        const unsigned long long pc0 = SC_DIAG_CLOCK(prof);
        SC_DIAG_DRAIN(prof);
        const unsigned long long pcw = SC_DIAG_CLOCK(prof);
        if (prof && b == 0) pc_first = pcw - pc_begin;
        walked += 4;
        int bsz = sc_cull_compact<true>(st, rect, __int_as_float(batch_start + lane), 0.f, xyoa_s, bck_s, col_s);
        const unsigned long long pc1 = SC_DIAG_CLOCK(prof);
        st.advance(in, flatten_ids, batch_start + 2 * B + lane, range_end, N);
        if (SC_DIAG_BIT(dbg, 1)) bsz = 0;
        const unsigned long long pc2 = SC_DIAG_CLOCK(prof);
        if (bsz > 0) {
            auto blend = [&](const float4& a, const float4& bc, const float4& c) {
                const float dy = a.y - px.py;
                const float bdy = sc_row_b(a.w, dy), qdy = sc_row_q(bc.y, dy);
                const int sidx = __float_as_int(bc.z);
#pragma unroll
                for (int p = 0; p < NP; ++p) {
                    const ScPairAlpha pa = sc_pair_alpha(a.x, bc.x, a.z, bdy, qdy, pxp[p]);
                    const sc_f2 al = pa.al;
                    const bool v0 = pa.v0, v1 = pa.v1;
                    const sc_f2 nT = __builtin_elementwise_fma(-al, T2[p], T2[p]);
                    const bool t0 = v0 && (nT.x <= SC_T_EPS), t1 = v1 && (nT.y <= SC_T_EPS);
                    const bool b0 = v0 != t0, b1 = v1 != t1;
                    const sc_f2 ae = sc_f2{b0 ? al.x : 0.f, b1 ? al.y : 0.f};
                    const sc_f2 vis = ae * T2[p];
                    T2[p] = __builtin_elementwise_fma(-ae, T2[p], T2[p]);
                    pxp[p] = sc_f2{t0 ? INF : pxp[p].x, t1 ? INF : pxp[p].y};
#pragma unroll
                    for (int h = 0; h < 2; ++h) {
                        const float vh = h ? vis.y : vis.x;
                        acc[2 * p + h][0] = __fmaf_rn(c.x, vh, acc[2 * p + h][0]);
                        acc[2 * p + h][1] = __fmaf_rn(c.y, vh, acc[2 * p + h][1]);
                        acc[2 * p + h][2] = __fmaf_rn(c.z, vh, acc[2 * p + h][2]);
                        if constexpr (CDIM > 3) acc[2 * p + h][3] = __fmaf_rn(c.w, vh, acc[2 * p + h][3]);
                    }
                    if (TRACK) {
                        cur[2 * p] = b0 ? sidx : cur[2 * p];
                        cur[2 * p + 1] = b1 ? sidx : cur[2 * p + 1];
                    }
                }
            };
            walked += sc_walk_batch(xyoa_s, bck_s, col_s, bsz, blend, all_done);
        }
        if (prof) {
            const unsigned long long pc3 = SC_DIAG_CLOCK(prof);
            pc_stage += pc2 - pc1; pc_issue += pc1 - pcw; pc_blend += pc3 - pc2; pc_batches += 1; pc_splats += (unsigned long long)bsz;
        }
    }
    if (PLANAR) {
        float Tv[PPL];
#pragma unroll
        for (int k = 0; k < PPL; ++k) Tv[k] = (k & 1) ? T2[k >> 1].y : T2[k >> 1].x;
        const bool v4 = PPL == 4 && (width & 3) == 0 && inside[PPL - 1];
        const bool v2 = PPL >= 2 && (width & 1) == 0;
        auto put = [&](float* base, const float* v) {
            if (PPL == 4 && v4) { *reinterpret_cast<float4*>(base) = make_float4(v[0], v[1], v[2], v[3 < PPL ? 3 : 0]); return; }
#pragma unroll
            for (int j = 0; j + 1 < PPL; j += 2) {
                if (v2 && inside[j + 1]) *reinterpret_cast<float2*>(base + j) = make_float2(v[j], v[j + 1]);
                else { if (inside[j]) base[j] = v[j]; if (inside[j + 1]) base[j + 1] = v[j + 1]; }
            }
        };
        float al[PPL];
#pragma unroll
        for (int k = 0; k < PPL; ++k) al[k] = 1.0f - Tv[k];
        put(render_alphas + pix0, al);
#pragma unroll
        for (int d = 0; d < CDIM; ++d) {
            float v[PPL];
#pragma unroll
            for (int k = 0; k < PPL; ++k) v[k] = backgrounds ? acc[k][d] + Tv[k] * backgrounds[cam * CDIM + d] : acc[k][d];
            put(render_colors + ppix0 + d * plane, v);
        }
    } else
#pragma unroll
    for (int k = 0; k < PPL; ++k) {
        if (!inside[k]) continue;
        const float Tk = (k & 1) ? T2[k >> 1].y : T2[k >> 1].x;
        const int64_t pix = pix0 + k;
        render_alphas[pix] = 1.0f - Tk;
        float o[CDIM];
#pragma unroll
        for (int d = 0; d < CDIM; ++d) o[d] = acc[k][d];
        if (backgrounds) {
#pragma unroll
            for (int d = 0; d < CDIM; ++d) o[d] += Tk * backgrounds[cam * CDIM + d];
        }
        if (ED) o[CDIM - 1] = o[CDIM - 1] / fmaxf(1.0f - Tk, 1e-10f);
        sc_store_pixel<CDIM>(render_colors, pix, o);
        if (TRACK) last_ids[pix] = cur[k];
    }
    if (tile_work && lane == 0) tile_work[tflat] = walked;
#ifdef SC_DIAG
    const int prow = tflat * 2 + (NSUB == 1 ? 0 : sub);
    if (prof && lane == 0 && prow < SC_PHASE_ROWS) {
        const unsigned long long pc_end = SC_DIAG_CLOCK(prof);
        unsigned long long* row = g_sc_phase_cycles[prow];
        row[0] += pc_end - pc_begin; row[1] += pc_stage; row[2] += pc_issue; row[3] += pc_blend;
        row[4] += 1ull; row[5] += pc_batches; row[6] += pc_splats; row[7] += pc_first;
        row[8] += SC_DIAG_REALTIME(prof) - pr_begin;
    }
#endif
}

template <int CDIM, bool TRACK, bool PACKED = false, bool ED = false, bool PLANAR = false>
__global__ __launch_bounds__(64) void raster_fwd_wave_kernel(
    const float* __restrict__ means2d, const float* __restrict__ conics,
    const float* __restrict__ colors, const float* __restrict__ opacities,
    const float* __restrict__ backgrounds, const uint8_t* __restrict__ tile_masks, int N,
    int width, int height, int tile_width, int tile_height, int total_tiles,
    const int32_t* __restrict__ isect_offsets, const int32_t* __restrict__ flatten_ids, int n_isects,
    float* __restrict__ render_colors, float* __restrict__ render_alphas,
    int32_t* __restrict__ last_ids, int map_mode, const int32_t* __restrict__ order,
    int32_t* __restrict__ tile_work SC_DIAG_PARAM(dbg)) {
    __shared__ float4 xyoa_s[SC_WALK_B + 1];
    __shared__ float4 bck_s[SC_WALK_B + 1];
    __shared__ float4 col_s[SC_WALK_B + 1];
    int tflat = blockIdx.x, kind = 0;
    if (order && tile_work)
        tile_work += (size_t)sc_clamp_view_slot(order[total_tiles + total_tiles / 8 + 8 + total_tiles + 1]) * total_tiles;
    if (order) {
        const int item = order[blockIdx.x];
        if (item < 0) return;
        tflat = item >> 2;
        kind = item & 3;
        if (tflat >= total_tiles || kind == 3) return;
    } else {
        if (tflat >= total_tiles) return;
        if (map_mode == 0) {
            const int nwg = gridDim.x, bid = blockIdx.x;
            const int xcd = bid & 7, idx = bid >> 3, q = nwg >> 3, r = nwg & 7;
            tflat = (xcd < r ? xcd * (q + 1) : r * (q + 1) + (xcd - r) * q) + idx;
        }
    }
    if (kind == 0)
        raster_item<CDIM, TRACK, 1, PACKED, ED, PLANAR>(means2d, conics, colors, opacities, backgrounds, tile_masks, N, width, height,
                                    tile_width, tile_height, total_tiles, isect_offsets, flatten_ids, n_isects,
                                    render_colors, render_alphas, last_ids, tflat, 0, xyoa_s, bck_s, col_s, tile_work
                                    SC_DIAG_ARG(dbg));
    else
        raster_item<CDIM, TRACK, 2, PACKED, ED, PLANAR>(means2d, conics, colors, opacities, backgrounds, tile_masks, N, width, height,
                                    tile_width, tile_height, total_tiles, isect_offsets, flatten_ids, n_isects,
                                    render_colors, render_alphas, last_ids, tflat, kind - 1, xyoa_s, bck_s, col_s,
                                    tile_work SC_DIAG_ARG(dbg));
}

}

int g_sc_raster_map = 1;
int g_sc_raster_hint_blend = 3;
int g_sc_raster_split = 50;

int sc_tile_order_fwd_items(int total_tiles) { return total_tiles + total_tiles / 8 + 8; }

extern "C" int sc_tile_order_len(int total_tiles) {
    return total_tiles < 0 ? 0 : sc_tile_order_fwd_items(total_tiles) + total_tiles + 2;
}

static int rasterize_fwd_impl(const float* means2d, const float* conics, const float* colors,
                              const float* opacities, const float* backgrounds,
                              const uint8_t* tile_masks, int C, int N, int D, int width, int height,
                              int tile_size, int tile_width, int tile_height,
                              const int32_t* isect_offsets, const int32_t* flatten_ids,
                              int64_t n_isects, float* render_colors, float* render_alphas,
                              int32_t* last_ids, const int32_t* tile_order, int32_t* tile_work,
                              sc_stream_t stream, int epilogue) {
    if (C < 0 || N < 0 || D < 1 || D > SC_MAX_CDIM || width <= 0 || height <= 0) return SC_EINVAL;
    if (tile_size < 1 || tile_size > 32 || tile_width <= 0 || tile_height <= 0) return SC_EINVAL;
    if (n_isects < 0 || n_isects > 0x7fffffffLL) return SC_EINVAL;
    if ((int64_t)tile_width * tile_size < width || (int64_t)tile_height * tile_size < height) return SC_EINVAL;
    if (C == 0) return SC_OK;
    if (!isect_offsets || !render_colors || !render_alphas) return SC_EINVAL;
    const bool packed = (epilogue & 2) != 0;
    if (n_isects > 0 && (!means2d || !flatten_ids || (!packed && (!conics || !colors || !opacities)))) return SC_EINVAL;
    if (C > 65535 || tile_height > 65535) return SC_EINVAL;
    dim3 grid(tile_width, tile_height, C);
    if ((int64_t)C * N > 0x7fffffffLL) return SC_EINVAL;
    const int NS = C * N;
    const int variant = g_sc_raster_fwd_variant;
    if ((epilogue & 3) && !(variant >= 3 && tile_size == 16 && D == 4)) return SC_EUNSUPPORTED;
    if ((epilogue & 4) && !(variant >= 3 && tile_size == 16 && (D == 3 || D == 4))) return SC_EUNSUPPORTED;
    if (packed && last_ids) return SC_EUNSUPPORTED;
    const bool ed = (epilogue & 1) != 0;
    const bool planar = (epilogue & 4) != 0;
    if (planar && (packed || ed || last_ids)) return SC_EUNSUPPORTED;
    if (variant >= 3 && tile_size == 16 && (D == 3 || D == 4)) {
        if ((int64_t)C * tile_width * tile_height >= (1 << 29)) return SC_EINVAL;
        const int total_tiles = C * tile_width * tile_height;
        const int n_blocks = tile_order ? sc_tile_order_fwd_items(total_tiles) : total_tiles;
        if (ed && last_ids) return SC_EUNSUPPORTED;
#define SC_LAUNCH_WAVE(CD, TR, PK, EDP, ...)                                                                        \
    hipLaunchKernelGGL((raster_fwd_wave_kernel<CD, TR, PK, EDP, ##__VA_ARGS__>), dim3(n_blocks), dim3(64), 0, sc_s(stream), means2d, \
                       conics, colors, opacities, backgrounds, tile_masks, NS, width, height, tile_width,           \
                       tile_height, total_tiles, isect_offsets, flatten_ids, (int)n_isects, render_colors,         \
                       render_alphas, last_ids, g_sc_raster_map, tile_order, tile_work SC_DIAG_ARG(g_sc_debug[1] & 0xff))
        if (planar) { if (D == 4) SC_LAUNCH_WAVE(4, false, false, false, true); else SC_LAUNCH_WAVE(3, false, false, false, true); }
        else if (packed) { if (ed) SC_LAUNCH_WAVE(4, false, true, true); else SC_LAUNCH_WAVE(4, false, true, false); }
        else if (D == 4) {
            if (ed) SC_LAUNCH_WAVE(4, false, false, true);
            else if (last_ids) SC_LAUNCH_WAVE(4, true, false, false);
            else SC_LAUNCH_WAVE(4, false, false, false);
        } else { if (last_ids) SC_LAUNCH_WAVE(3, true, false, false); else SC_LAUNCH_WAVE(3, false, false, false); }
#undef SC_LAUNCH_WAVE
        SC_LAUNCH_CHECK();
        return SC_OK;
    }
    dim3 block(tile_size, tile_size);
    const size_t shmem = (size_t)tile_size * tile_size * 40;
    if (D == 4)
        hipLaunchKernelGGL(raster_fwd_ref_kernel<4>, grid, block, shmem, sc_s(stream), means2d, conics, colors,
                           opacities, backgrounds, tile_masks, NS, D, width, height, tile_size, tile_width,
                           tile_height, isect_offsets, flatten_ids, (int)n_isects, render_colors,
                           render_alphas, last_ids);
    else if (D == 3)
        hipLaunchKernelGGL(raster_fwd_ref_kernel<3>, grid, block, shmem, sc_s(stream), means2d, conics, colors,
                           opacities, backgrounds, tile_masks, NS, D, width, height, tile_size, tile_width,
                           tile_height, isect_offsets, flatten_ids, (int)n_isects, render_colors,
                           render_alphas, last_ids);
    else
        hipLaunchKernelGGL(raster_fwd_ref_kernel<0>, grid, block, shmem, sc_s(stream), means2d, conics, colors,
                           opacities, backgrounds, tile_masks, NS, D, width, height, tile_size, tile_width,
                           tile_height, isect_offsets, flatten_ids, (int)n_isects, render_colors,
                           render_alphas, last_ids);
    SC_LAUNCH_CHECK();
    return SC_OK;
}

extern "C" int sc_rasterize_fwd(const float* means2d, const float* conics, const float* colors,
                                const float* opacities, const float* backgrounds,
                                const uint8_t* tile_masks, int C, int N, int D, int width, int height,
                                int tile_size, int tile_width, int tile_height,
                                const int32_t* isect_offsets, const int32_t* flatten_ids,
                                int64_t n_isects, float* render_colors, float* render_alphas,
                                int32_t* last_ids, const int32_t* tile_order, int32_t* tile_work,
                                sc_stream_t stream) {
    return rasterize_fwd_impl(means2d, conics, colors, opacities, backgrounds, tile_masks, C, N, D, width, height,
                              tile_size, tile_width, tile_height, isect_offsets, flatten_ids, n_isects,
                              render_colors, render_alphas, last_ids, tile_order, tile_work, stream, 0);
}

extern "C" int sc_rasterize_fwd_planar(const float* means2d, const float* conics, const float* colors,
                                       const float* opacities, const float* backgrounds,
                                       const uint8_t* tile_masks, int C, int N, int D, int width, int height,
                                       int tile_size, int tile_width, int tile_height,
                                       const int32_t* isect_offsets, const int32_t* flatten_ids,
                                       int64_t n_isects, float* render_colors, float* render_alphas,
                                       const int32_t* tile_order, int32_t* tile_work, sc_stream_t stream) {
    return rasterize_fwd_impl(means2d, conics, colors, opacities, backgrounds, tile_masks, C, N, D, width, height,
                              tile_size, tile_width, tile_height, isect_offsets, flatten_ids, n_isects,
                              render_colors, render_alphas, nullptr, tile_order, tile_work, stream, 4);
}

extern "C" int sc_rasterize_fwd_ed(const float* means2d, const float* conics, const float* colors,
                                   const float* opacities, const float* backgrounds,
                                   const uint8_t* tile_masks, int C, int N, int D, int width, int height,
                                   int tile_size, int tile_width, int tile_height,
                                   const int32_t* isect_offsets, const int32_t* flatten_ids,
                                   int64_t n_isects, float* render_colors, float* render_alphas,
                                   const int32_t* tile_order, int32_t* tile_work, sc_stream_t stream) {
    return rasterize_fwd_impl(means2d, conics, colors, opacities, backgrounds, tile_masks, C, N, D, width, height,
                              tile_size, tile_width, tile_height, isect_offsets, flatten_ids, n_isects,
                              render_colors, render_alphas, nullptr, tile_order, tile_work, stream, 1);
}


extern "C" int sc_rasterize_fwd_packed(const float* records, const float* backgrounds, const uint8_t* tile_masks,
                                       int C, int N, int width, int height, int tile_width, int tile_height,
                                       const int32_t* isect_offsets, const int32_t* flatten_ids, int64_t n_isects,
                                       float* render_colors, float* render_alphas, const int32_t* tile_order,
                                       int32_t* tile_work, int depth_normalise, sc_stream_t stream) {
    if (g_sc_raster_fwd_variant < 3) return SC_EUNSUPPORTED;
    if (records && ((uintptr_t)records & 15)) return SC_EINVAL;
    return rasterize_fwd_impl(records, nullptr, nullptr, nullptr, backgrounds, tile_masks, C, N, 4, width, height, 16,
                              tile_width, tile_height, isect_offsets, flatten_ids, n_isects, render_colors,
                              render_alphas, nullptr, tile_order, tile_work, stream,
                              2 | (depth_normalise ? 1 : 0));
}
```

### street_crafter_amd/csrc/raster_walk.h

```cpp
#pragma once
#include "raster_common.h"

constexpr int SC_WALK_B = 64;

struct ScTileId { int cam, txi, tyi; };
__device__ __forceinline__ ScTileId sc_tile_id(int tflat, int tile_width, int tile_height) {
    const int tiles_per_cam = tile_width * tile_height;
    ScTileId t;
    t.cam = tflat / tiles_per_cam;
    const int tile_id = tflat - t.cam * tiles_per_cam;
    t.tyi = tile_id / tile_width;
    t.txi = tile_id - t.tyi * tile_width;
    return t;
}
struct ScRect { float x0, x1, y0, y1; };
__device__ __forceinline__ ScRect sc_tile_rect(const ScTileId& t, int row0, int rows, int width, int height) {
    ScRect r;
    r.x0 = (float)(t.txi * 16) + 0.5f;
    r.y0 = (float)(t.tyi * 16 + row0) + 0.5f;
    r.x1 = (float)min(t.txi * 16 + 15, width - 1) + 0.5f;
    r.y1 = (float)min(t.tyi * 16 + row0 + rows - 1, height - 1) + 0.5f;
    return r;
}
template <int NSUB>
// ... 11 lines not shown
        py_i = t.tyi * 16 + (sub * ROWS + lane / LPR);
        py = (float)py_i + 0.5f;
#pragma unroll
        for (int k = 0; k < PPL; ++k) inside[k] = (px0_i + k < width) && (py_i < height);
        pix0 = ((int64_t)t.cam * height + py_i) * width + px0_i;
    }
    __device__ __forceinline__ ScRect rect(const ScTileId& t, int sub, int width, int height) const {
        return sc_tile_rect(t, sub * ROWS, ROWS, width, height);
    }
    __device__ __forceinline__ sc_f2 x_pair(int p, int px0, float off) const {
        return sc_f2{inside[2 * p] ? (float)(px0 + 2 * p) + 0.5f : off,
                     inside[2 * p + 1] ? (float)(px0 + 2 * p + 1) + 0.5f : off};
    }
};

struct ScSplatArrays { const float* means2d; const float* conics; const float* colors; const float* opacities; };
struct ScNoExtra { __device__ __forceinline__ void operator()(int) const {} };

template <int CDIM, bool PACKED = false>
struct ScStage {
    float2 xy;
    float a, b, c, op;
    float4 col;
    bool live;
    int g_next;
    __device__ __forceinline__ void clear() {
        xy = make_float2(0.f, 0.f);
        a = b = c = op = 0.f;
        col = make_float4(0.f, 0.f, 0.f, 0.f);
    }
    template <class Extra = ScNoExtra>
    __device__ __forceinline__ void load(int g, const ScSplatArrays& in, Extra&& extra = Extra()) {
        live = g >= 0;
        if (!live) return;
        if (PACKED) {
            const float4* rec = reinterpret_cast<const float4*>(in.means2d) + (int64_t)g * 3;
            const float4 q0 = rec[0], q1 = rec[1], q2 = rec[2];
            xy = make_float2(q0.x, q0.y);
            a = q0.z; b = q0.w; c = q1.x;
            op = q1.y;
            col = make_float4(q1.z, q1.w, q2.x, CDIM > 3 ? q2.y : 0.f);
            return;
        }
        xy = *reinterpret_cast<const float2*>(in.means2d + (int64_t)g * 2);
        const float* cn = in.conics + (int64_t)g * 3;
        a = cn[0]; b = cn[1]; c = cn[2];
        op = in.opacities[g];
        const float* cl = in.colors + (int64_t)g * CDIM;
        col = make_float4(cl[0], cl[1], cl[2], CDIM > 3 ? cl[3] : 0.f);
        extra(g);
    }
    static __device__ __forceinline__ int id_at(const int32_t* __restrict__ flatten_ids, int idx, int end, int n_splats) {
        return (idx < end) ? sc_safe_id(flatten_ids[idx], n_splats) : -1;
    }
    template <class Extra = ScNoExtra>
    __device__ __forceinline__ void advance(const ScSplatArrays& in, const int32_t* __restrict__ flatten_ids, int idx2,
                                            int end, int n_splats, Extra&& extra = Extra()) {
        load(g_next, in, extra);
        g_next = id_at(flatten_ids, idx2, end, n_splats);
    }
};

__device__ __forceinline__ float sc_guard_a2(float A2) { return A2 == 0.f ? 1e-37f : A2; }
struct ScAlwaysOpen { __device__ __forceinline__ bool operator()() const { return true; } };
template <bool GUARD_A2, class Stage, class Open = ScAlwaysOpen>
__device__ __forceinline__ int sc_cull_compact(const Stage& st, const ScRect& r, float w2, float w3, float4* xyoa_s,
                                               float4* bck_s, float4* col_s, Open&& open = Open()) {
    __syncthreads();
    bool keep = false;
    if (st.live)
        keep = open() && !splat_misses_rect(st.a, st.b, st.c, st.op, r.x0 - st.xy.x, r.x1 - st.xy.x, r.y0 - st.xy.y,
                                            r.y1 - st.xy.y);
    const unsigned long long m = __ballot(keep);
    if (keep) {
        const int slot = __popcll(m & sc_lanemask_lt());
        const ScSplat sp = sc_prescale(st.xy.x, st.xy.y, st.a, st.b, st.c, st.op);
        xyoa_s[slot] = make_float4(sp.mx, sp.my, sp.lop, sp.B2);
        bck_s[slot] = make_float4(GUARD_A2 ? sc_guard_a2(sp.A2) : sp.A2, sp.C2, w2, w3);
        col_s[slot] = st.col;
    }
    __syncthreads();
    return __popcll(m);
}

struct ScPairAlpha { sc_f2 sg, al; bool v0, v1; };
__device__ __forceinline__ ScPairAlpha sc_pair_alpha(float mx, float A2, float lop, float bdy, float qdy, sc_f2 px) {
    ScPairAlpha r;
    const sc_f2 dx = sc_f2{mx, mx} - px;
    const sc_f2 tt = __builtin_elementwise_fma(sc_f2{A2, A2}, dx, sc_f2{bdy, bdy});
    r.sg = __builtin_elementwise_fma(tt, dx, sc_f2{qdy, qdy});
    const sc_f2 e = sc_f2{lop, lop} - r.sg;
    r.al = sc_f2{fminf(SC_ALPHA_MAX, __builtin_amdgcn_exp2f(e.x)), fminf(SC_ALPHA_MAX, __builtin_amdgcn_exp2f(e.y))};
    r.v0 = sc_valid(r.sg.x, r.al.x);
    r.v1 = sc_valid(r.sg.y, r.al.y);
    return r;
}

enum ScMark { MARK_X, MARK_TSIGN };
template <ScMark MARK, int ND, bool TRACK, int W>
__device__ __forceinline__ void sc_blend_step(const sc_f2 al, const bool v0, const bool v1, const float4& c, sc_f2& T,
                                              sc_f2& px, float (&ac0)[W], float (&ac1)[W], int idx, int& last0,
                                              int& last1) {
    const sc_f2 nT = __builtin_elementwise_fma(-al, T, T);
    const bool t0 = v0 && (nT.x <= SC_T_EPS), t1 = v1 && (nT.y <= SC_T_EPS);
    const bool b0 = v0 != t0, b1 = v1 != t1;
    const sc_f2 ae = sc_f2{b0 ? al.x : 0.f, b1 ? al.y : 0.f};
// ... 66 lines not shown
```

### street_crafter_amd/isect.py

```python
from __future__ import annotations

import collections
import math
import os
import threading
import weakref
from typing import Optional, Tuple

import torch
from torch import Tensor

from . import _lib
from .lazy import LazyTensor as _LazyTensor


def _env_on(name: str, default: bool = True) -> bool:
    v = os.environ.get(name)
    return default if v is None or v == "" else v not in ("0", "false", "False", "off", "no")


class _Switches:
    __slots__ = ("tile_order", "lazy_ids", "view_slots", "packed_records", "defer_isect", "planar_out", "fused_train")

    def __init__(self):
        self.tile_order = _env_on("SC_TILE_ORDER")
        self.lazy_ids = _env_on("SC_LAZY_IDS")
        self.view_slots = _env_on("SC_VIEW_SLOTS")
        self.packed_records = _env_on("SC_PACKED_RECORDS")
        self.defer_isect = _env_on("SC_DEFER_ISECT")
        self.planar_out = _env_on("SC_PLANAR_OUTPUT")
        self.fused_train = _env_on("SC_FUSED_TRAIN", False)

    def flip(self, name: str, value: bool) -> bool:
        prev = getattr(self, name)
        setattr(self, name, bool(value))
        return prev


def _predicted_capacities(history, bucket_cap) -> Tuple[int, int, int]:
    mi, mr, ms = map(max, zip(*history))
    ms_pred = ms + ms // 8 + 64
    if ms <= bucket_cap < ms_pred:
        ms_pred = bucket_cap
    return mi + mi // 8 + 4096, mr + mr // 8 + 4096, ms_pred


class _OperatorState:
    KEYS_MAX = 64

    def __init__(self):
        self.prediction, self.history, self.last_meta = {}, {}, {}
        self.history_len = 8
        self.tile_work, self.view_registry = {}, {}
        self.stats = {"calls": 0, "speculative_ok": 0, "exact_relaunch": 0}
        self.bucket_cap = {}
        self.sched_sizes = {}

    def tables(self):
        return (("predictions", self.prediction), ("history", self.history), ("last_meta", self.last_meta),
                ("tile_work", self.tile_work), ("view_registry", self.view_registry))

    def reset(self, idx=None) -> dict:
        dropped = {}
        for name, table in self.tables():
            keys = [k for k in table if idx is None or (k[0] if isinstance(k, tuple) else k) == idx]
            for k in keys:
                table.pop(k, None)
            dropped[name] = len(keys)
        return dropped

    def record(self, key, sizes, bucket_cap):
        hist = self.history.get(key)
        if hist is None:
            hist = self.history[key] = collections.deque(maxlen=self.history_len)
            while len(self.history) > self.KEYS_MAX:
                old = next(iter(self.history))
                for table in (self.history, self.prediction, self.last_meta):
                    table.pop(old, None)
        hist.append(sizes)
        self.last_meta[key] = sizes
        self.prediction[key] = _predicted_capacities(hist, bucket_cap)


_SWITCH = _Switches()
_STATE = _OperatorState()

_ISECT_MODE = {"mode": "bin"}


def set_isect_mode(mode: str) -> str:
    assert mode in ("bin", "radix")
    prev = _ISECT_MODE["mode"]
    _ISECT_MODE["mode"] = mode
    return prev


def set_lazy_isect_ids(enabled: bool) -> bool:
    return _SWITCH.flip("lazy_ids", enabled)


def set_deferred_isect(enabled: bool) -> bool:
    return _SWITCH.flip("defer_isect", enabled)


def _p(t: Optional[Tensor]):
    return None if t is None else t.data_ptr()


_RAW_STREAM = getattr(torch._C, "_cuda_getCurrentRawStream", None)


def _stream(t: Tensor):
    if _RAW_STREAM is not None:
        return _RAW_STREAM(t.device.index if t.device.index is not None else torch.cuda.current_device())
    return torch.cuda.current_stream(t.device).cuda_stream


def _req(t: Tensor, name: str, dtype=torch.float32):
    if type(t) is Tensor and t.dtype is dtype and t.is_cuda and t.is_contiguous():
        return t
    if not isinstance(t, Tensor):
        raise TypeError(f"{name} must be a torch.Tensor, got {type(t)}")
    if not t.is_cuda:
        raise RuntimeError(f"{name} must live on a HIP device (got {t.device}); "
                           "street_crafter_amd has no CPU path")
    if t.dtype != dtype:
        raise TypeError(f"{name} must be {dtype}, got {t.dtype}")
    return t.contiguous()


def _ws(nbytes: int, device) -> Tensor:
    return torch.empty(max(int(nbytes), 256), dtype=torch.uint8, device=device)


_WARNED = set()


def _warn_once(key, msg, *args):
    if key not in _WARNED:
        _WARNED.add(key)
        import logging
        logging.getLogger("street_crafter_amd").warning(msg, *args)


@torch.no_grad()
def isect_tiles(means2d: Tensor, radii: Tensor, depths: Tensor, tile_size: int, tile_width: int,
                tile_height: int, sort: bool = True, packed: bool = False,
                n_cameras: Optional[int] = None, camera_ids: Optional[Tensor] = None,
                gaussian_ids: Optional[Tensor] = None) -> Tuple[Tensor, Tensor, Tensor]:
    if packed:
        raise NotImplementedError("packed=True is not supported (reference passes packed=False)")
    view_cams = getattr(means2d, "_sc_viewmats", None)
    means2d = _req(means2d.detach() if means2d.requires_grad else means2d, "means2d")
    radii = _req(radii, "radii", torch.int32)
    depths = _req(depths.detach() if depths.requires_grad else depths, "depths")
    C, N = radii.shape
    assert means2d.shape == (C, N, 2), means2d.shape
    assert depths.shape == (C, N), depths.shape
    if n_cameras is not None:
        assert int(n_cameras) == C, (n_cameras, C)
    st = _stream(means2d)
    mode = _ISECT_MODE["mode"] if sort else "radix"
    if mode == "bin":
        res = _isect_tiles_bin(means2d, radii, depths, C, N, tile_size, tile_width, tile_height, st,
                               viewmats=view_cams, defer=True)
        if res is not None:
            return res[:3]
    return _isect_tiles_radix(means2d, radii, depths, C, N, tile_size, tile_width, tile_height, sort, st)


def _isect_tiles_radix(means2d, radii, depths, C, N, tile_size, tile_width, tile_height, sort, st):
    lib = _lib.load()
    dev = means2d.device
    tiles_per_gauss = torch.empty((C, N), dtype=torch.int32, device=dev)
    total_dev = torch.empty(1, dtype=torch.int64, device=dev)
    wsb = lib.sc_isect_workspace_bytes(C * N)
    ws = _ws(wsb, dev)
    _lib.check(lib.sc_isect_count(_p(means2d), _p(radii), C, N, int(tile_size), int(tile_width),
                                  int(tile_height), _p(tiles_per_gauss), _p(total_dev), _p(ws), ws.numel(), st),
               "sc_isect_count")
    n_isects = int(total_dev.item())
    _check_isect_count(n_isects, C, N, tile_width, tile_height)
    isect_ids = torch.empty(n_isects, dtype=torch.int64, device=dev)
    flatten_ids = torch.empty(n_isects, dtype=torch.int32, device=dev)
    if n_isects:
        _lib.check(lib.sc_isect_emit(_p(means2d), _p(radii), _p(depths), C, N, int(tile_size), int(tile_width),
                                     int(tile_height), _p(tiles_per_gauss), n_isects, _p(isect_ids),
                                     _p(flatten_ids), _p(ws), ws.numel(), st), "sc_isect_emit")
        if sort:
            n_tiles = tile_width * tile_height
            tile_bits = int(math.floor(math.log2(n_tiles))) + 1
            cam_bits = int(math.floor(math.log2(C))) + 1
            tmp_k = torch.empty_like(isect_ids)
            tmp_v = torch.empty_like(flatten_ids)
            sws = _ws(lib.sc_radix_sort_workspace_bytes(n_isects), dev)
            _lib.check(lib.sc_radix_sort_pairs_u64_i32(_p(isect_ids), _p(flatten_ids), _p(tmp_k), _p(tmp_v),
                                                       n_isects, 32 + tile_bits + cam_bits, _p(sws),
                                                       sws.numel(), st), "sc_radix_sort_pairs_u64_i32")
    return tiles_per_gauss, isect_ids, flatten_ids


def _check_isect_count(n_isects, C, N, tile_width, tile_height):
    if n_isects > 0x7fffffff:
        raise RuntimeError(f"isect_tiles: {n_isects} tile intersections exceed the int32 range of isect_offsets "
                           f"({C} cameras x {N} Gaussians on {tile_width}x{tile_height} tiles); render fewer "
                           "cameras per call or cull the scene")


def _view_registry(dev) -> Optional[Tensor]:
    if not (_SWITCH.view_slots and _SWITCH.tile_order):
        return None
    reg = _STATE.view_registry.get(dev.index)
    if reg is None:
        reg = _STATE.view_registry[dev.index] = torch.zeros(_lib.load().sc_view_registry_words(), dtype=torch.int32, device=dev)
    return reg


def _tile_work(dev, C, N, tile_width, tile_height) -> Tensor:
# ... 13 lines not shown

    def __init__(self, host):
        self.host, self.view, self.ptr, self.seq, self.pending = host, host.numpy(), host.data_ptr(), 0, None

    def settle_pending(self, warn_key, warn_msg):
        pending, self.pending = self.pending and self.pending(), None
        if pending is not None:
            try:
                pending.resolve()
            except Exception as e:
                _warn_once(warn_key, warn_msg, type(e).__name__, e)


_PINNED_META = threading.local()


class _PendingIsect:
    __slots__ = ("settle", "flat_ref", "ids_ref", "done", "lock", "flat_plain", "error", "__weakref__")

    def __init__(self, settle):
        self.settle, self.flat_ref, self.ids_ref = settle, None, None
        self.done, self.lock, self.flat_plain, self.error = False, threading.Lock(), None, None

    def resolve(self, _tensor=None):
        with self.lock:
            if self.done:
                return
            if self.error is not None:
                raise self.error
            settle, self.settle = self.settle, None
            try:
                fids, ids_buf, after = settle()
            except BaseException as e:
                self.error = e
                raise
            self.flat_plain = fids
            with torch._C.DisableTorchFunctionSubclass():
                for ref, src in ((self.flat_ref, fids), (self.ids_ref, ids_buf)):
                    t = ref() if ref is not None else None
                    if t is not None and src is not None:
                        t.set_(src)
                        t.__dict__["_sc_resolve"] = None
            self.done = True
            if after is not None:
                after()


def _bin_launch_ran(capacities, n_isects, n_records, max_super) -> bool:
    return n_isects <= capacities[0] and n_records <= capacities[1] and max_super <= capacities[2]


class _BinCall:
    __slots__ = ("b", "st", "dev", "inputs", "depths", "C", "N", "grid", "offsets", "meta_dev", "ws0", "slot", "seq",
                 "eager_ids", "key", "pred", "ids", "fids", "flat", "n_isects", "ids_ref")

    def __init__(self, b, st, inputs, C, N, grid, offsets, meta_dev, ws0, slot, eager_ids):
        self.b, self.st, self.dev = b, st, offsets.device
        self.inputs, self.depths, self.C, self.N, self.grid = inputs, inputs[2], C, N, grid
        self.offsets, self.meta_dev, self.ws0, self.slot, self.seq = offsets, meta_dev, ws0, slot, slot.seq
        self.eager_ids, self.key = eager_ids, (self.dev.index, C, N, *grid)
        self.pred = self.ids = self.fids = self.flat = self.n_isects = self.ids_ref = None

    def read_meta(self):
        if self.b.wait_i64(self.slot.ptr + 32, self.seq, 2_000_000) != 0:
            torch.cuda.ExternalStream(self.st, device=self.dev).synchronize()
            return tuple(int(v) for v in self.meta_dev.cpu().tolist())
        return tuple(map(int, self.slot.view[:4]))

    def launch(self, capacities):
        rc, self.ids, self.fids = self.b.isect_bin_sort(
            *self.inputs, *self.grid, self.offsets, self.meta_dev, self.ws0, int(capacities[0]), int(capacities[1]),
            int(capacities[2]), bool(self.eager_ids), self.st)
        return rc

    def settle(self):
        n_isects, _, n_records, max_super = self.read_meta()
        C, N, st, (_, tile_width, tile_height) = self.C, self.N, self.st, self.grid
        _check_isect_count(n_isects, C, N, tile_width, tile_height)
        ran = self.pred is not None and _bin_launch_ran(self.pred, n_isects, n_records, max_super)
        _STATE.stats["calls"] += 1
        if self.pred is not None:
            _STATE.stats["speculative_ok" if ran else "exact_relaunch"] += 1
        if not ran:
            if self.pred is not None:
                _lib.check(_lib.load().sc_isect_bin_reset_cursors(_p(self.ws0), C * N, C, tile_width, tile_height, st),
                           "sc_isect_bin_reset_cursors")
            if _stream(self.offsets) != st:
                with torch.cuda.stream(torch.cuda.ExternalStream(st, device=self.dev)):
                    rc = self.launch((n_isects, n_records, max_super))
            else:
                rc = self.launch((n_isects, n_records, max_super))
            if rc == -3:
                return None
            _lib.check(rc, "sc_isect_bin_sort")
        cap = _STATE.bucket_cap.get("v") or _STATE.bucket_cap.setdefault("v", int(_lib.load().sc_isect_bin_bucket_capacity()))
        _STATE.record(self.key, (n_isects, n_records, max_super), cap)
        self.flat, self.n_isects = self.fids[:n_isects], n_isects
        self.inputs = self.meta_dev = self.ws0 = None
        return n_isects

    def fill_ids(self, buf):
        cur = _stream(buf)
        if cur != self.st:
            ev = torch.cuda.Event()
            ev.record(torch.cuda.ExternalStream(self.st, device=self.dev))
            torch.cuda.current_stream(self.dev).wait_event(ev)
        _lib.check(_lib.load().sc_isect_ids_rebuild(self.flat.data_ptr(), self.offsets.data_ptr(), self.depths.data_ptr(),
                                                    self.C, self.N, self.grid[1], self.grid[2], self.n_isects,
                                                    buf.data_ptr(), cur), "sc_isect_ids_rebuild")

    def file_offsets(self, isect_ids=None):
        isect_ids = self.ids_ref() if isect_ids is None else isect_ids
        if isect_ids is not None:
            with torch._C.DisableTorchFunctionSubclass():
                isect_ids._sc_offsets = (self.offsets, self.C, self.grid[1], self.grid[2], isect_ids._version)

    def deferred(self):
        pending = _PendingIsect(self.settle_deferred)
        flatten_ids = _LazyTensor(self.fids[:0], None, pending.resolve)
        isect_ids = _LazyTensor(torch.empty(0, dtype=torch.int64, device=self.dev), self.fill_ids, pending.resolve)
        pending.flat_ref, pending.ids_ref = weakref.ref(flatten_ids), weakref.ref(isect_ids)
        self.slot.pending, self.ids_ref = weakref.ref(pending), pending.ids_ref
        self.file_offsets(isect_ids)
        return isect_ids, flatten_ids

    def settle_deferred(self):
        n_isects = self.settle()
        if n_isects is not None:
            return self.flat, torch.empty(n_isects, dtype=torch.int64, device=self.dev), self.file_offsets
        with torch.cuda.stream(torch.cuda.ExternalStream(self.st, device=self.dev)):
            _, ids, flat = _isect_tiles_radix(*self.inputs, self.C, self.N, *self.grid, True, self.st)
        isect_ids = self.ids_ref()
        if isect_ids is not None:
            isect_ids.__dict__["_sc_fill"] = None
        return flat, ids, self.file_offsets


def _isect_tiles_bin(means2d, radii, depths, C, N, tile_size, tile_width, tile_height, st, want_ids=True,
                     viewmats=None, defer=False):
    dev = means2d.device
    b = _lib.binding()
    slots = _PINNED_META.__dict__.setdefault("slots", {})
    slot = slots.get(dev.index)
    if slot is None:
        slot = slots[dev.index] = _MetaSlot(torch.zeros(8, dtype=torch.int64, pin_memory=True))
    slot.settle_pending("settle_prev", "isect_tiles: settling the previous, never observed call failed (%s: %s); its own "
                        "tensors raise the error when they are looked at")
    slot.seq += 1
    grid = (int(tile_size), int(tile_width), int(tile_height))
    want_order = _SWITCH.tile_order and grid[0] == 16
    work = _tile_work(dev, C, N, tile_width, tile_height) if want_order else None
    registry = None
    if (want_order and viewmats is not None and viewmats.device == dev and viewmats.dtype == torch.float32
            and viewmats.is_contiguous() and viewmats.shape == (C, 4, 4)):
        registry = _view_registry(dev)
    if registry is None:
        viewmats = None
    rc, tiles_per_gauss, offsets, meta_dev, ws0, order = b.isect_bin_count(
        means2d, radii, depths, *grid, work, viewmats, registry, bool(want_order), slot.ptr, slot.seq, st)
    if want_order:
        offsets._sc_sched = (order, work)
    if rc == -3:
        return None
    if rc:
        _lib.check(rc, "sc_isect_bin_count")
    eager_ids = want_ids and not _SWITCH.lazy_ids
    call = _BinCall(b, st, (means2d, radii, depths), C, N, grid, offsets, meta_dev, ws0, slot, eager_ids)
    pred = _STATE.prediction.get(call.key)
    if pred is not None:
        rc = call.launch(pred)
        if rc == 0:
            call.pred = pred
        elif rc != -3:
            _lib.check(rc, "sc_isect_bin_sort")
    if defer and call.pred is not None and want_ids and not eager_ids and _SWITCH.defer_isect:
        return (tiles_per_gauss, *call.deferred(), offsets)
    n_isects = call.settle()
    if n_isects is None:
        return None
    isect_ids = None
    if want_ids:
        isect_ids = (call.ids[:n_isects] if eager_ids
                     else _LazyTensor(torch.empty(n_isects, dtype=torch.int64, device=dev), call.fill_ids))
        call.file_offsets(isect_ids)
    return tiles_per_gauss, isect_ids, call.flat, offsets


@torch.no_grad()
def isect_offset_encode(isect_ids: Tensor, n_cameras: int, tile_width: int, tile_height: int) -> Tensor:
    lib = _lib.load()
    cached = getattr(isect_ids, "_sc_offsets", None)
    if cached is not None and cached[1:4] == (int(n_cameras), int(tile_width), int(tile_height)):
        if (isect_ids.__dict__.get("_sc_touched") is None if type(isect_ids) is _LazyTensor
                else isect_ids._version == cached[4]):
            return cached[0]
    isect_ids = _req(isect_ids, "isect_ids", torch.int64)
    dev = isect_ids.device
    offsets = torch.empty((n_cameras, tile_height, tile_width), dtype=torch.int32, device=dev)
    _lib.check(lib.sc_isect_offsets(_p(isect_ids), isect_ids.numel(), int(n_cameras), int(tile_width),
                                    int(tile_height), _p(offsets), _stream(isect_ids)), "sc_isect_offsets")
    return offsets
```

### street_crafter_amd/rendering.py

```python
from __future__ import annotations

import math
from typing import Optional, Tuple

import torch
from torch import Tensor

from . import _lib
from .lazy import LazyTensor as _LazyTensor
from .isect import (_ISECT_MODE, _PINNED_META, _RAW_STREAM, _STATE, _SWITCH, _BinCall, _MetaSlot,
                    _OperatorState, _PendingIsect, _Switches, _bin_launch_ran, _check_isect_count, _isect_tiles_bin,
                    _isect_tiles_radix, _p, _req, _stream, _tile_work, _view_registry, _warn_once, _ws,
                    isect_offset_encode, isect_tiles, set_deferred_isect, set_isect_mode, set_lazy_isect_ids)

__all__ = ["fully_fused_projection", "isect_tiles", "isect_offset_encode", "spherical_harmonics",
           "rasterize_to_pixels", "rasterization"]


class _NoGradCtx:
    needs_input_grad = (False,) * 16

    def save_for_backward(self, *tensors):
        pass

    def mark_non_differentiable(self, *tensors):
        pass

    def __setattr__(self, name, value):
        pass


_NO_GRAD_CTX = _NoGradCtx()
_EMPTY = {}


def _needs_grad(*args) -> bool:
    return torch.is_grad_enabled() and any(isinstance(a, Tensor) and a.requires_grad for a in args)


def _call(fn, *args):
    if _needs_grad(*args):
        return fn.apply(*args)
    return fn.forward(_NO_GRAD_CTX, *args)


_NATIVE_AUTOGRAD = {"on": True}


def set_native_autograd(enabled: bool) -> bool:
    prev, _NATIVE_AUTOGRAD["on"] = _NATIVE_AUTOGRAD["on"], bool(enabled)
    return prev


def _native():
    if not _NATIVE_AUTOGRAD["on"] or _BACKWARD_PROBE["events"] is not None or _RAW_STREAM is None:
        return None
    return _lib.fast()


_BACKWARD_PROBE = {"events": None}


def set_backward_probe(events):
    prev, _BACKWARD_PROBE["events"] = _BACKWARD_PROBE["events"], events
    return prev

# ... 178 lines not shown
        if not tab:
            _RASTER_SIDE.pop(idx, None)
    else:
        tab[key] = side
    return prev


def reset_state(device=None) -> dict:
    idx = None if device is None else (device if isinstance(device, int) else torch.device(device).index)
    for d, slot in getattr(_PINNED_META, "slots", {}).items():
        if idx is None or d == idx:
            slot.settle_pending("settle_reset", "reset_state: settling a never observed isect_tiles call failed (%s: %s)")
    return _STATE.reset(idx)


def _sched_of(isect_offsets, n_tiles):
    sched = getattr(isect_offsets, "_sc_sched", None) if _SWITCH.tile_order else None
    if sched is None:
        return None, None
    want = _STATE.sched_sizes.get(n_tiles)
    if want is None:
        if len(_STATE.sched_sizes) > 64:
            _STATE.sched_sizes.clear()
        want = _STATE.sched_sizes[n_tiles] = (_lib.load().sc_view_slots() * n_tiles, _lib.load().sc_tile_order_len(n_tiles))
    if sched[1].numel() != want[0] or sched[0].device != isect_offsets.device or sched[0].numel() != want[1]:
        return None, None
    return sched


class _Rasterize(torch.autograd.Function):
    @staticmethod
    def forward(ctx, means2d, conics, colors, opacities, backgrounds, masks, width, height, tile_size,
                isect_offsets, flatten_ids, absgrad, means2d_obj):
        C = opacities.shape[0]
        D = colors.shape[-1]
        th, tw = isect_offsets.shape[1], isect_offsets.shape[2]
        dev = means2d.device
        needs_bwd = any(ctx.needs_input_grad[:5])
        order, work = _sched_of(isect_offsets, C * tw * th)
        b = _lib.binding()
        st = _stream(means2d)
        side = cur = None
        if _RASTER_SIDE and not needs_bwd:
            tab = _RASTER_SIDE.get(dev.index)
            side = (tab.get(st) or tab.get(None)) if tab else None
            if side is not None:
                cur = torch.cuda.current_stream(dev)
                ev = torch.cuda.Event()
                ev.record(cur)
                side.wait_event(ev)
                st = side.cuda_stream
        rc = -3
        last_ids = None
        if _SWITCH.planar_out and not needs_bwd and int(tile_size) == 16 and D in (3, 4):
            rc, render_colors, render_alphas = b.rasterize_fwd_planar(
                means2d, conics, colors, opacities, backgrounds, masks, int(width), int(height), int(tile_size),
                isect_offsets, flatten_ids, order, work, st)
            if rc not in (0, -3):
                _lib.check(rc, "sc_rasterize_fwd_planar")
        if rc == -3:
            rc, render_colors, render_alphas, last_ids = b.rasterize_fwd(
                means2d, conics, colors, opacities, backgrounds, masks, int(width), int(height), int(tile_size),
                isect_offsets, flatten_ids, bool(needs_bwd), order, work, st)
            if rc:
                _lib.check(rc, "sc_rasterize_fwd")
        if side is not None:
            ev = torch.cuda.Event()
            ev.record(side)
            cur.wait_event(ev)
        e = _EMPTY.get(dev)
        if e is None:
            e = _EMPTY[dev] = torch.empty(0, device=dev)
        ctx.save_for_backward(means2d, conics, colors, opacities, backgrounds if backgrounds is not None else e,
                              masks if masks is not None else e, isect_offsets, flatten_ids, render_alphas,
                              last_ids if last_ids is not None else e)
        ctx.meta = (int(width), int(height), int(tile_size), bool(absgrad), backgrounds is not None,
                    masks is not None)
        ctx.means2d_obj = means2d_obj
        ctx.tile_order = order
        return render_colors, render_alphas

    @staticmethod
    def backward(ctx, v_render_colors, v_render_alphas):
        (means2d, conics, colors, opacities, backgrounds, masks, isect_offsets, flatten_ids, render_alphas,
         last_ids) = ctx.saved_tensors
        width, height, tile_size, absgrad, has_bg, has_mask = ctx.meta
        v_render_colors = v_render_colors.contiguous()
        v_render_alphas = v_render_alphas.contiguous()
        with _probe("rasterize_to_pixels_bwd"):
            rc, v_means2d, v_conics, v_colors, v_opacities, v_abs = _lib.binding().rasterize_bwd(
                means2d, conics, colors, opacities, backgrounds if has_bg else None, masks if has_mask else None,
                width, height, tile_size, isect_offsets, flatten_ids, render_alphas, last_ids, v_render_colors,
                v_render_alphas, bool(absgrad), ctx.tile_order, _stream(means2d))
        if rc:
            _lib.check(rc, "sc_rasterize_bwd")
        if absgrad:
            ctx.means2d_obj.tensor.absgrad = v_abs
        v_bg = None
        if has_bg and ctx.needs_input_grad[4]:
            v_bg = (v_render_colors * (1.0 - render_alphas)).sum(dim=(1, 2))
        return (v_means2d, v_conics, v_colors, v_opacities, v_bg, None, None, None, None, None, None, None, None)


class _AbsgradTarget:
    __slots__ = ("tensor",)

    def __init__(self, tensor):
        self.tensor = tensor


def rasterize_to_pixels(means2d: Tensor, conics: Tensor, colors: Tensor, opacities: Tensor,
                        image_width: int, image_height: int, tile_size: int, isect_offsets: Tensor,
                        flatten_ids: Tensor, backgrounds: Optional[Tensor] = None,
                        masks: Optional[Tensor] = None, packed: bool = False,
                        absgrad: bool = False) -> Tuple[Tensor, Tensor]:
    if packed:
        raise NotImplementedError("packed=True is not supported (reference passes packed=False)")
    caller_means2d = means2d
    means2d_c = _req(means2d, "means2d")
    conics = _req(conics, "conics")
    colors = _req(colors, "colors")
    opacities = _req(opacities, "opacities")
    isect_offsets = _req(isect_offsets, "isect_offsets", torch.int32)
    if type(flatten_ids) is _LazyTensor:
        flatten_ids = flatten_ids.plain()
    flatten_ids = _req(flatten_ids, "flatten_ids", torch.int32)
    C, N = opacities.shape
    D = colors.shape[-1]
    assert means2d_c.shape == (C, N, 2), means2d_c.shape
    assert conics.shape == (C, N, 3), conics.shape
    assert colors.shape == (C, N, D), colors.shape
    assert isect_offsets.ndim == 3 and isect_offsets.shape[0] == C, isect_offsets.shape
    th, tw = isect_offsets.shape[1], isect_offsets.shape[2]
    assert tw * tile_size >= image_width, "image_width must fit in tile_width * tile_size"
    assert th * tile_size >= image_height, "image_height must fit in tile_height * tile_size"
    if not 1 <= D <= 32:
        raise NotImplementedError(f"colour channels must be in 1..32, got {D}")
    if backgrounds is not None:
        backgrounds = _req(backgrounds, "backgrounds")
        assert backgrounds.shape == (C, D), backgrounds.shape
    if masks is not None:
        assert masks.shape == isect_offsets.shape, masks.shape
        if not masks.is_cuda:
            raise RuntimeError("masks must live on a HIP device")
        masks = masks.to(torch.uint8).contiguous()

    nat = _native() if _needs_grad(means2d_c, conics, colors, opacities, backgrounds) else None
    if nat is not None:
        order, work = _sched_of(isect_offsets, C * tw * th)
        return nat.rasterize_autograd(means2d_c, conics, colors, opacities, backgrounds, masks, int(image_width),
                                      int(image_height), int(tile_size), isect_offsets, flatten_ids, bool(absgrad), order,
                                      work, caller_means2d, _RAW_STREAM)
    return _call(_Rasterize, means2d_c, conics, colors, opacities, backgrounds, masks, int(image_width),
                            int(image_height), int(tile_size), isect_offsets, flatten_ids, bool(absgrad),
                            _AbsgradTarget(caller_means2d))


def camera_centers(viewmats: Tensor) -> Tensor:
    lib = _lib.load()
    viewmats = _req(viewmats, "viewmats")
    out = torch.empty((viewmats.shape[0], 3), dtype=torch.float32, device=viewmats.device)
    _lib.check(lib.sc_camera_centers(_p(viewmats), viewmats.shape[0], _p(out), _stream(viewmats)),
               "sc_camera_centers")
    return out


_FUSED_RASTERIZATION = True


def set_fused_rasterization(enabled: bool) -> bool:
    global _FUSED_RASTERIZATION
    prev, _FUSED_RASTERIZATION = _FUSED_RASTERIZATION, bool(enabled)
    return prev


def _fused_forward_ok(tensors, sh_degree, render_mode, tile_size, colors) -> bool:
    if not _FUSED_RASTERIZATION or sh_degree is None or render_mode not in ("RGB+D", "RGB+ED"):
        return False
    if tile_size != 16 or colors.dim() != 3 or colors.shape[-1] != 3:
        return False
    if torch.is_grad_enabled() and any(t is not None and t.requires_grad for t in tensors):
        return False
    return True


def set_fused_training(enabled: bool) -> bool:
    return _SWITCH.flip("fused_train", enabled)


def _fused_train_ok(leaves, cameras, sh_degree, render_mode, tile_size, colors) -> bool:
    if not _SWITCH.fused_train or not _FUSED_RASTERIZATION or sh_degree is None or render_mode not in ("RGB+D", "RGB+ED"):
        return False
    if tile_size != 16 or colors.dim() != 3 or colors.shape[-1] != 3:
        return False
    if not torch.is_grad_enabled() or not any(t.requires_grad for t in leaves):
        return False
    return not any(t is not None and t.requires_grad for t in cameras)


class _ProjectionSh(torch.autograd.Function):

    @staticmethod
    def forward(ctx, means, quats, scales, opacities, sh, viewmats, Ks, centers, sh_degree, width, height, eps2d,
                near_plane, far_plane, radius_clip, antialiased):
        rc, radii, means2d, depths, _, conics, opac, cols = _lib.binding().projection_sh_fwd(
            means, quats, scales, opacities, sh, viewmats, Ks, centers, int(sh_degree), int(width), int(height),
            float(eps2d), float(near_plane), float(far_plane), float(radius_clip), bool(antialiased), False,
            _stream(means))
# ... 256 lines not shown
```

Before: 3175.

## Rasterize directly from super-tile buckets and defer per-tile flatten_ids emission

Adds a bucket path where the bin sort writes sorted gaussian ids per super-tile instead of expanding them into per-tile flatten_ids. The forward rasterizer reads the super-tile buckets directly. Per-tile flatten_ids are only emitted lazily through a new emit kernel when some consumer actually needs them. This is meant to remove the cost of writing and re-reading the full per-tile intersection list in forward-only rendering. In exchange, each tile now scans a larger super-tile list, and the lazy-tensor bookkeeping and fallback paths get more complex.

```diff
diff --git a/include/street_crafter_amd.h b/include/street_crafter_amd.h
--- a/include/street_crafter_amd.h
+++ b/include/street_crafter_amd.h
@@ -78,6 +78,15 @@
 int sc_isect_ids_rebuild(const int32_t* flatten_ids, const int32_t* isect_offsets, const float* depths,
                          int C, int N, int tile_width, int tile_height, int64_t n_isects,
                          int64_t* isect_ids, sc_stream_t stream);
+int64_t sc_isect_bin_super_tiles(int C, int tile_width, int tile_height);
+int sc_isect_bin_sort_buckets(const float* means2d, const int32_t* radii, const float* depths, int C, int N,
+                              int tile_size, int tile_width, int tile_height, const int64_t* meta_dev,
+                              void* count_workspace, int64_t capacity, int64_t rec_capacity, int64_t super_capacity,
+                              int32_t* super_ids, int32_t* super_offsets, void* workspace, size_t ws_bytes,
+                              sc_stream_t stream);
+int sc_isect_emit_tiles(const int32_t* super_ids, const int32_t* super_offsets, const int32_t* isect_offsets,
+                        int C, int tile_width, int tile_height, int64_t n_records, int64_t n_isects,
+                        int32_t* flatten_ids, sc_stream_t stream);
 int sc_isect_bin_reset_cursors(void* count_workspace, int64_t CN, int C, int tile_width, int tile_height,
                                sc_stream_t stream);
 
@@ -264,6 +273,13 @@
                             const int32_t* isect_offsets, const int32_t* flatten_ids, int64_t n_isects,
                             float* render_colors, float* render_alphas,
                             const int32_t* tile_order, int32_t* tile_work, sc_stream_t stream);
+int sc_rasterize_fwd_buckets(const float* means2d, const float* conics, const float* colors,
+                             const float* opacities, const float* backgrounds, const uint8_t* tile_masks,
+                             int C, int N, int D, int width, int height, int tile_size,
+                             int tile_width, int tile_height,
+                             const int32_t* super_offsets, const int32_t* super_ids, int64_t n_records,
+                             float* render_colors, float* render_alphas,
+                             const int32_t* tile_order, int32_t* tile_work, int planar, sc_stream_t stream);
 int sc_records_unpack(const float* records, int64_t CN, float* conics, float* opacities, float* colors4,
                       sc_stream_t stream);
 int sc_rasterize_fwd_ed(const float* means2d, const float* conics, const float* colors,
diff --git a/street_crafter_amd/_ctypes_binding.py b/street_crafter_amd/_ctypes_binding.py
--- a/street_crafter_amd/_ctypes_binding.py
+++ b/street_crafter_amd/_ctypes_binding.py
@@ -75,6 +75,27 @@
     return rc, ids, fids
 
 
+def isect_bin_sort_buckets(means2d, radii, depths, tile_size, tile_width, tile_height, meta_dev, ws0, capacity,
+                           rec_capacity, super_capacity, stream):
+    lib = _lib.load()
+    C, N = radii.shape
+    dev = means2d.device
+    sids = torch.empty(rec_capacity, dtype=torch.int32, device=dev)
+    soffs = torch.empty(max(int(lib.sc_isect_bin_super_tiles(C, int(tile_width), int(tile_height))), 0) + 1,
+                        dtype=torch.int32, device=dev)
+    ws = _ws(lib.sc_isect_bin_workspace_bytes(C * N, C, tile_width, tile_height, rec_capacity), dev)
+    rc = lib.sc_isect_bin_sort_buckets(_p(means2d), _p(radii), _p(depths), C, N, int(tile_size), int(tile_width),
+                                       int(tile_height), _p(meta_dev), _p(ws0), capacity, rec_capacity, super_capacity,
+                                       _p(sids), _p(soffs), _p(ws), ws.numel(), stream)
+    return rc, sids, soffs
+
+
+def isect_emit_tiles(super_ids, super_offsets, offsets, n_records, flatten_ids, stream):
+    C, th, tw = offsets.shape
+    return _lib.load().sc_isect_emit_tiles(_p(super_ids), _p(super_offsets), _p(offsets), C, tw, th, int(n_records),
+                                           flatten_ids.numel(), _p(flatten_ids), stream)
+
+
 def wait_i64(addr, value, timeout_us):
     return _lib.load().sc_wait_i64(addr, value, timeout_us)
 
@@ -126,6 +147,22 @@
                                              _p(offsets), _p(flatten_ids), flatten_ids.numel(), _p(planes),
                                              _p(render_alphas), _p(order), _p(work), stream)
     return rc, planes.permute(0, 2, 3, 1), render_alphas
+
+
+def rasterize_fwd_buckets(means2d, conics, colors, opacities, backgrounds, masks, width, height, tile_size, tile_width,
+                          tile_height, super_offsets, super_ids, n_records, order, work, planar, stream):
+    C, N = opacities.shape
+    D = colors.shape[-1]
+    dev = means2d.device
+    shape = (C, D, height, width) if planar else (C, height, width, D)
+    out = torch.empty(shape, dtype=torch.float32, device=dev)
+    render_alphas = torch.empty((C, height, width, 1), dtype=torch.float32, device=dev)
+    rc = _lib.load().sc_rasterize_fwd_buckets(_p(means2d), _p(conics), _p(colors), _p(opacities), _p(backgrounds),
+                                              _p(masks), C, N, D, int(width), int(height), int(tile_size),
+                                              int(tile_width), int(tile_height), _p(super_offsets), _p(super_ids),
+                                              int(n_records), _p(out), _p(render_alphas), _p(order), _p(work),
+                                              1 if planar else 0, stream)
+    return rc, (out.permute(0, 2, 3, 1) if planar else out), render_alphas
 
 
 def rasterize_fwd_groups(means2d, conics, colors, opacities, group_ids, n_groups, width, height, tile_size, offsets,
diff --git a/street_crafter_amd/_lib.py b/street_crafter_amd/_lib.py
--- a/street_crafter_amd/_lib.py
+++ b/street_crafter_amd/_lib.py
@@ -92,6 +92,15 @@
                                     c_i32p, C.c_void_p, C.c_size_t, c_stream]),
     "sc_isect_ids_rebuild": (C.c_int, [c_i32p, c_i32p, c_f32p, C.c_int, C.c_int, C.c_int, C.c_int, C.c_int64, c_i64p,
                                        c_stream]),
+    "sc_isect_bin_super_tiles": (C.c_int64, [C.c_int, C.c_int, C.c_int]),
+    "sc_isect_bin_sort_buckets": (C.c_int, [c_f32p, c_i32p, c_f32p, C.c_int, C.c_int, C.c_int, C.c_int, C.c_int,
+                                            c_i64p, C.c_void_p, C.c_int64, C.c_int64, C.c_int64, c_i32p, c_i32p,
+                                            C.c_void_p, C.c_size_t, c_stream]),
+    "sc_isect_emit_tiles": (C.c_int, [c_i32p, c_i32p, c_i32p, C.c_int, C.c_int, C.c_int, C.c_int64, C.c_int64, c_i32p,
+                                      c_stream]),
+    "sc_rasterize_fwd_buckets": (C.c_int, [c_f32p, c_f32p, c_f32p, c_f32p, c_f32p, c_u8p, C.c_int, C.c_int, C.c_int,
+                                           C.c_int, C.c_int, C.c_int, C.c_int, C.c_int, c_i32p, c_i32p, C.c_int64,
+                                           c_f32p, c_f32p, c_i32p, c_i32p, C.c_int, c_stream]),
     "sc_isect_bin_reset_cursors": (C.c_int, [C.c_void_p, C.c_int64, C.c_int, C.c_int, C.c_int, c_stream]),
     "sc_isect_offsets": (C.c_int, [c_i64p, C.c_int64, C.c_int, C.c_int, C.c_int, c_i32p, c_stream]),
     "sc_sh_fwd": (C.c_int, [C.c_int, c_f32p, c_f32p, c_u8p, C.c_int64, C.c_int, c_f32p, c_stream]),
diff --git a/street_crafter_amd/csrc/binding.cpp b/street_crafter_amd/csrc/binding.cpp
--- a/street_crafter_amd/csrc/binding.cpp
+++ b/street_crafter_amd/csrc/binding.cpp
@@ -124,6 +124,33 @@
     return py::make_tuple(rc, ids, fids);
 }
 
+py::tuple isect_bin_sort_buckets(const Tensor& means2d, const Tensor& radii, const Tensor& depths, int64_t tile_size,
+                                 int64_t tile_width, int64_t tile_height, const Tensor& meta_dev, const Tensor& ws0,
+                                 int64_t capacity, int64_t rec_capacity, int64_t super_capacity, int64_t stream) {
+    const int64_t C = radii.size(0), N = radii.size(1);
+    Tensor sids = at::empty({rec_capacity}, i32(means2d));
+    const int64_t nsb = std::max<int64_t>(sc_isect_bin_super_tiles((int)C, (int)tile_width, (int)tile_height), 0);
+    Tensor soffs = at::empty({nsb + 1}, i32(means2d));
+    size_t wsb = sc_isect_bin_workspace_bytes(C * N, (int)C, (int)tile_width, (int)tile_height, rec_capacity);
+    if (wsb < 256) wsb = 256;
+    Tensor ws = at::empty({(int64_t)wsb}, u8(means2d));
+    const int rc = sc_isect_bin_sort_buckets(fp(means2d), ip(radii), fp(depths), (int)C, (int)N, (int)tile_size,
+                                             (int)tile_width, (int)tile_height,
+                                             static_cast<const int64_t*>(meta_dev.data_ptr()), ws0.data_ptr(), capacity,
+                                             rec_capacity, super_capacity, static_cast<int32_t*>(sids.data_ptr()),
+                                             static_cast<int32_t*>(soffs.data_ptr()), ws.data_ptr(), wsb, S(stream));
+    return py::make_tuple(rc, sids, soffs);
+}
+
+int isect_emit_tiles(const Tensor& super_ids, const Tensor& super_offsets, const Tensor& offsets, int64_t n_records,
+                     const Tensor& flatten_ids, int64_t stream) {
+    req(super_ids, at::kInt, "super_ids"); req(super_offsets, at::kInt, "super_offsets");
+    req(offsets, at::kInt, "isect_offsets"); req(flatten_ids, at::kInt, "flatten_ids");
+    return sc_isect_emit_tiles(ip(super_ids), ip(super_offsets), ip(offsets), (int)offsets.size(0), (int)offsets.size(2),
+                               (int)offsets.size(1), n_records, flatten_ids.numel(),
+                               static_cast<int32_t*>(flatten_ids.data_ptr()), S(stream));
+}
+
 int wait_i64(int64_t addr, int64_t value, int64_t timeout_us) {
     py::gil_scoped_release nogil;
     return sc_wait_i64(reinterpret_cast<const int64_t*>(static_cast<uintptr_t>(addr)), value, timeout_us);
@@ -201,6 +228,27 @@
                                            order ? ip(*order) : nullptr,
                                            work ? static_cast<int32_t*>(work->data_ptr()) : nullptr, S(stream));
     return py::make_tuple(rc, planes.permute({0, 2, 3, 1}), ra);
+}
+py::tuple rasterize_fwd_buckets(const Tensor& means2d, const Tensor& conics, const Tensor& colors, const Tensor& opacities,
+                                const OptT& backgrounds, const OptT& masks, int64_t width, int64_t height, int64_t tile_size,
+                                int64_t tile_width, int64_t tile_height, const Tensor& super_offsets, const Tensor& super_ids,
+                                int64_t n_records, const OptT& order, const OptT& work, bool planar, int64_t stream) {
+    req(means2d, at::kFloat, "means2d"); req(conics, at::kFloat, "conics"); req(colors, at::kFloat, "colors");
+    req(opacities, at::kFloat, "opacities"); req(super_offsets, at::kInt, "super_offsets"); req(super_ids, at::kInt, "super_ids");
+    const int64_t C = opacities.size(0), N = opacities.size(1), D = colors.size(-1);
+    TORCH_CHECK(n_records >= 0 && n_records <= super_ids.numel(), "n_records exceeds super_ids");
+    TORCH_CHECK(super_offsets.numel() == sc_isect_bin_super_tiles((int)C, (int)tile_width, (int)tile_height) + 1,
+                "super_offsets must hold one bound per super-tile + 1");
+    Tensor out = planar ? at::empty({C, D, height, width}, f32(means2d)) : at::empty({C, height, width, D}, f32(means2d));
+    Tensor ra = at::empty({C, height, width, 1}, f32(means2d));
+    const int rc = sc_rasterize_fwd_buckets(fp(means2d), fp(conics), fp(colors), fp(opacities), fpo(backgrounds),
+                                            masks ? static_cast<const uint8_t*>(masks->data_ptr()) : nullptr, (int)C, (int)N,
+                                            (int)D, (int)width, (int)height, (int)tile_size, (int)tile_width,
+                                            (int)tile_height, ip(super_offsets), ip(super_ids), n_records, fpw(out), fpw(ra),
+                                            order ? ip(*order) : nullptr,
+                                            work ? static_cast<int32_t*>(work->data_ptr()) : nullptr, planar ? 1 : 0,
+                                            S(stream));
+    return py::make_tuple(rc, planar ? out.permute({0, 2, 3, 1}) : out, ra);
 }
 py::tuple rasterize_fwd_groups(const Tensor& means2d, const Tensor& conics, const Tensor& colors, const Tensor& opacities,
                                const Tensor& group_ids, int64_t n_groups, int64_t width, int64_t height, int64_t tile_size,
@@ -897,11 +945,14 @@
     m.def("projection_bwd", &projection_bwd);
     m.def("isect_bin_count", &isect_bin_count);
     m.def("isect_bin_sort", &isect_bin_sort);
+    m.def("isect_bin_sort_buckets", &isect_bin_sort_buckets);
+    m.def("isect_emit_tiles", &isect_emit_tiles);
     m.def("wait_i64", &wait_i64);
     m.def("sh_fwd", &sh_fwd);
     m.def("sh_bwd", &sh_bwd);
     m.def("rasterize_fwd", &rasterize_fwd);
     m.def("rasterize_fwd_planar", &rasterize_fwd_planar);
+    m.def("rasterize_fwd_buckets", &rasterize_fwd_buckets);
     m.def("rasterize_fwd_groups", &rasterize_fwd_groups);
     m.def("rasterize_fwd_layers", &rasterize_fwd_layers);
     m.def("rasterize_fwd_groups_ids", &rasterize_fwd_groups_ids);
diff --git a/street_crafter_amd/csrc/isect_bin.hip b/street_crafter_amd/csrc/isect_bin.hip
--- a/street_crafter_amd/csrc/isect_bin.hip
+++ b/street_crafter_amd/csrc/isect_bin.hip
@@ -694,8 +694,8 @@
 __device__ __forceinline__ void sort_segment(
     const uint2* __restrict__ recs, int n, int sb, const int* tb, int cap, const Geo& g,
     const int32_t* __restrict__ offsets, int n_tbuckets, int64_t n_isects, int tile_bits,
-    unsigned char* smem, int64_t* __restrict__ isect_ids, int32_t* __restrict__ flatten_ids, unsigned* totals_out
-    SC_DIAG_PARAM(dbg)) {
+    unsigned char* smem, int64_t* __restrict__ isect_ids, int32_t* __restrict__ flatten_ids, unsigned* totals_out,
+    int32_t* __restrict__ super_out SC_DIAG_PARAM(dbg)) {
     constexpr int WAVES = THREADS / 64, NC = THREADS;
     unsigned long long* B = reinterpret_cast<unsigned long long*>(smem);
     unsigned short* order = reinterpret_cast<unsigned short*>(B + cap);
@@ -838,6 +838,10 @@
         order[r] = (unsigned short)p;
     }
     __syncthreads();
+    if (super_out) {
+        for (int i = t; i < n; i += THREADS) super_out[i] = (int32_t)(unsigned)B[order[i]];
+        return;
+    }
     emit_tiles<THREADS>(B, order, n, sb, g, offsets, n_tbuckets, n_isects, tile_bits, tb, table, isect_ids,
                            flatten_ids, totals SC_DIAG_ARG(dbg));
     if (totals_out) {
@@ -849,7 +853,7 @@
 __device__ __forceinline__ void sort_heavy_segment(
     const uint2* __restrict__ src, uint2* __restrict__ dst, int n, int sb, const int* tb_in, int cap, const Geo& g,
     const int32_t* __restrict__ offsets, int n_tbuckets, int64_t n_isects, int tile_bits, unsigned char* smem,
-    int64_t* __restrict__ isect_ids, int32_t* __restrict__ flatten_ids) {
+    int64_t* __restrict__ isect_ids, int32_t* __restrict__ flatten_ids, int32_t* __restrict__ super_out) {
     unsigned long long* B = reinterpret_cast<unsigned long long*>(smem);
     unsigned long long* table = reinterpret_cast<unsigned long long*>(smem + (size_t)cap * 8);
     __shared__ unsigned tot[4];
@@ -860,8 +864,10 @@
         const unsigned long long K = rec_key60(r);
         int rank = 0;
         for (int j = 0; j < n; ++j) rank += rec_key60(src[j]) < K ? 1 : 0;
-        dst[rank] = r;
-    }
+        if (super_out) super_out[rank] = (int32_t)r.y;
+        else dst[rank] = r;
+    }
+    if (super_out) return;
     if (t < 4) tbr[t] = tb_in[t];
     __threadfence();
     __syncthreads();
@@ -889,7 +895,8 @@
     const int32_t* __restrict__ soffsets, int n_sbuckets, int n_tbuckets,
     Geo g, const int32_t* __restrict__ offsets, const int64_t* __restrict__ meta, int64_t capacity,
     int64_t rec_capacity, int64_t super_capacity, int tile_bits, int cap,
-    int64_t* __restrict__ isect_ids, int32_t* __restrict__ flatten_ids SC_DIAG_PARAM(dbg)) {
+    int64_t* __restrict__ isect_ids, int32_t* __restrict__ flatten_ids, int32_t* __restrict__ super_ids,
+    int32_t* __restrict__ super_offsets SC_DIAG_PARAM(dbg)) {
     extern __shared__ __align__(16) unsigned char smem[];
     if (meta[0] > capacity || meta[2] > rec_capacity || meta[3] > super_capacity) return;
     __shared__ int tb_s[4];
@@ -901,21 +908,54 @@
         __syncthreads();
         if (sg->heavy)
             sort_heavy_segment(temp + start, records_rw + start, sn, ssb, tb_s, cap, g, offsets, n_tbuckets,
-                               meta[0], tile_bits, smem, isect_ids, flatten_ids);
+                               meta[0], tile_bits, smem, isect_ids, flatten_ids, super_ids ? super_ids + start : nullptr);
         else
             sort_segment<SS_THREADS, SS_RPT>(temp + start, sn, ssb, tb_s, cap, g, offsets, n_tbuckets, meta[0], tile_bits,
-                                             smem, isect_ids, flatten_ids, nullptr SC_DIAG_ARG(dbg));
+                                             smem, isect_ids, flatten_ids, nullptr, super_ids ? super_ids + start : nullptr
+                                             SC_DIAG_ARG(dbg));
         return;
     }
     const int sb = (int)blockIdx.x - seg_bound;
     const int s = soffsets[sb];
     const int e = (sb + 1 < n_sbuckets) ? soffsets[sb + 1] : (int)meta[2];
     const int n = e - s;
+    if (super_offsets && threadIdx.x == 0) {
+        super_offsets[sb] = s;
+        if (sb + 1 == n_sbuckets) super_offsets[n_sbuckets] = e;
+    }
     if (n <= 0 || n > cap) return;
     if (threadIdx.x < 4) tb_s[threadIdx.x] = 0;
     __syncthreads();
     sort_segment<THREADS, RPT>(records + s, n, sb, tb_s, cap, g, offsets, n_tbuckets, meta[0], tile_bits, smem, isect_ids,
-                               flatten_ids, nullptr SC_DIAG_ARG(dbg));
+                               flatten_ids, nullptr, super_ids ? super_ids + s : nullptr SC_DIAG_ARG(dbg));
+}
+
+constexpr int EB_THREADS = 256;
+constexpr int EB_CHUNK = 2048;
+__global__ __launch_bounds__(EB_THREADS) void emit_from_buckets_kernel(
+    const int32_t* __restrict__ super_ids, const int32_t* __restrict__ super_offsets, int n_tbuckets, Geo g,
+    const int32_t* __restrict__ offsets, int64_t n_isects, int n_records, int tile_bits,
+    int32_t* __restrict__ flatten_ids) {
+    __shared__ unsigned long long B[EB_CHUNK];
+    __shared__ unsigned long long table[(EB_CHUNK / EB_THREADS + 1) * (EB_THREADS / 64) + 8];
+    __shared__ unsigned tot[4];
+    __shared__ int tbr[4];
+    const int t = threadIdx.x, sb = blockIdx.x;
+    const int s = min(max(super_offsets[sb], 0), n_records);
+    const int e = min(max(super_offsets[sb + 1], s), n_records);
+    if (t < 4) tbr[t] = 0;
+    __syncthreads();
+    for (int c0 = s; c0 < e; c0 += EB_CHUNK) {
+        const int m = min(EB_CHUNK, e - c0);
+        for (int i = t; i < m; i += EB_THREADS) B[i] = (unsigned long long)(unsigned)super_ids[c0 + i];
+        __syncthreads();
+        int tbl[4] = {tbr[0], tbr[1], tbr[2], tbr[3]};
+        emit_tiles<EB_THREADS>(B, nullptr, m, sb, g, offsets, n_tbuckets, n_isects, tile_bits, tbl, table, nullptr,
+                               flatten_ids, tot SC_DIAG_ARG(0));
+        __syncthreads();
+        if (t < 4) tbr[t] += (int)tot[t];
+        __syncthreads();
+    }
 }
 
 __global__ __launch_bounds__(256) void isect_ids_rebuild_kernel(
@@ -1344,12 +1384,12 @@
     return SC_OK;
 }
 
-extern "C" int sc_isect_bin_sort(const float* means2d, const int32_t* radii, const float* depths, int C,
-                                 int N, int tile_size, int tile_width, int tile_height,
-                                 const int32_t* isect_offsets, const int64_t* meta_dev,
-                                 void* count_workspace, int64_t capacity, int64_t rec_capacity,
-                                 int64_t super_capacity, int64_t* isect_ids, int32_t* flatten_ids,
-                                 void* workspace, size_t ws_bytes, sc_stream_t stream) {
+static int bin_sort_impl(const float* means2d, const int32_t* radii, const float* depths, int C,
+                         int N, int tile_size, int tile_width, int tile_height,
+                         const int32_t* isect_offsets, const int64_t* meta_dev,
+                         void* count_workspace, int64_t capacity, int64_t rec_capacity,
+                         int64_t super_capacity, int64_t* isect_ids, int32_t* flatten_ids, int32_t* super_ids,
+                         int32_t* super_offsets, bool buckets, void* workspace, size_t ws_bytes, sc_stream_t stream) {
     if (C < 0 || N < 0 || tile_size <= 0 || tile_width <= 0 || tile_height <= 0 || capacity < 0 ||
         rec_capacity < 0 || super_capacity < 0)
         return SC_EINVAL;
@@ -1361,9 +1401,8 @@
     const bool big = super_capacity > SS_MAX_CAP;
     int cap = big ? SS_MAX_CAP : (int)((super_capacity + 255) / 256 * 256);
     if (cap < 256) cap = 256;
-    if (!means2d || !radii || !depths || !isect_offsets || !meta_dev || !count_workspace || !flatten_ids ||
-        !workspace)
-        return SC_EINVAL;
+    if (!means2d || !radii || !depths || !meta_dev || !count_workspace || !workspace) return SC_EINVAL;
+    if (buckets ? (!super_ids || !super_offsets) : (!isect_offsets || !flatten_ids)) return SC_EINVAL;
     if (ws_bytes < sc_isect_bin_workspace_bytes(CN, C, tile_width, tile_height, rec_capacity)) return SC_EWORKSPACE;
     hipStream_t s = sc_s(stream);
     const BinLayout L = bin_layout(CN, C, N, tile_width, tile_height);
@@ -1404,7 +1443,7 @@
     hipLaunchKernelGGL((super_sort_kernel<THREADSP, RPTP>), dim3(GRID), dim3(THREADSP), LDSB, s,                              \
                        (const uint2*)records, records, (const uint2*)temp, (const Segment*)segs, (const unsigned*)n_segs, SEGB, \
                        soffsets, L.nsb, L.ntb, L.g, isect_offsets, meta_dev, capacity, rec_capacity, super_capacity, tile_bits,  \
-                       cap, isect_ids, flatten_ids SC_DIAG_ARG(g_sc_debug[2]))
+                       cap, isect_ids, flatten_ids, super_ids, super_offsets SC_DIAG_ARG(g_sc_debug[2]))
     if (!big && cap <= SS_SMALL_CAP)
         SC_LAUNCH_SORT(SS_SMALL_THREADS, SS_SMALL_RPT, (unsigned)L.nsb, sort_lds_bytes(cap, SS_SMALL_THREADS), 0);
     else
@@ -1413,3 +1452,45 @@
     SC_LAUNCH_CHECK();
     return SC_OK;
 }
+
+extern "C" int sc_isect_bin_sort(const float* means2d, const int32_t* radii, const float* depths, int C,
+                                 int N, int tile_size, int tile_width, int tile_height,
+                                 const int32_t* isect_offsets, const int64_t* meta_dev,
+                                 void* count_workspace, int64_t capacity, int64_t rec_capacity,
+                                 int64_t super_capacity, int64_t* isect_ids, int32_t* flatten_ids,
+                                 void* workspace, size_t ws_bytes, sc_stream_t stream) {
+    return bin_sort_impl(means2d, radii, depths, C, N, tile_size, tile_width, tile_height, isect_offsets, meta_dev,
+                         count_workspace, capacity, rec_capacity, super_capacity, isect_ids, flatten_ids, nullptr, nullptr,
+                         false, workspace, ws_bytes, stream);
+}
+
+extern "C" int64_t sc_isect_bin_super_tiles(int C, int tile_width, int tile_height) {
+    if (C < 0 || tile_width <= 0 || tile_height <= 0) return SC_EINVAL;
+    return (int64_t)C * ((tile_width + 1) >> 1) * ((tile_height + 1) >> 1);
+}
+
+extern "C" int sc_isect_bin_sort_buckets(const float* means2d, const int32_t* radii, const float* depths, int C,
+                                         int N, int tile_size, int tile_width, int tile_height, const int64_t* meta_dev,
+                                         void* count_workspace, int64_t capacity, int64_t rec_capacity,
+                                         int64_t super_capacity, int32_t* super_ids, int32_t* super_offsets,
+                                         void* workspace, size_t ws_bytes, sc_stream_t stream) {
+    return bin_sort_impl(means2d, radii, depths, C, N, tile_size, tile_width, tile_height, nullptr, meta_dev,
+                         count_workspace, capacity, rec_capacity, super_capacity, nullptr, nullptr, super_ids, super_offsets,
+                         true, workspace, ws_bytes, stream);
+}
+
+extern "C" int sc_isect_emit_tiles(const int32_t* super_ids, const int32_t* super_offsets, const int32_t* isect_offsets,
+                                   int C, int tile_width, int tile_height, int64_t n_records, int64_t n_isects,
+                                   int32_t* flatten_ids, sc_stream_t stream) {
+    if (C < 0 || tile_width <= 0 || tile_height <= 0 || n_records < 0 || n_isects < 0 || n_records > 0x7fffffffLL ||
+        n_isects > 0x7fffffffLL)
+        return SC_EINVAL;
+    if ((int64_t)C * tile_width * tile_height > BIN_MAX_TILES) return SC_EUNSUPPORTED;
+    if (C == 0 || n_records == 0 || n_isects == 0) return SC_OK;
+    if (!super_ids || !super_offsets || !isect_offsets || !flatten_ids) return SC_EINVAL;
+    const BinLayout L = bin_layout(0, C, 1, tile_width, tile_height);
+    hipLaunchKernelGGL(emit_from_buckets_kernel, dim3((unsigned)L.nsb), dim3(EB_THREADS), 0, sc_s(stream), super_ids,
+                       super_offsets, L.ntb, L.g, isect_offsets, n_isects, (int)n_records, sc_bits_for(L.g.T), flatten_ids);
+    SC_LAUNCH_CHECK();
+    return SC_OK;
+}
diff --git a/street_crafter_amd/csrc/raster_fwd.hip b/street_crafter_amd/csrc/raster_fwd.hip
--- a/street_crafter_amd/csrc/raster_fwd.hip
+++ b/street_crafter_amd/csrc/raster_fwd.hip
@@ -139,7 +139,7 @@
     const int32_t* __restrict__ isect_offsets, const int32_t* __restrict__ flatten_ids, int n_isects,
     float* __restrict__ render_colors, float* __restrict__ render_alphas,
     int32_t* __restrict__ last_ids, int tflat, int sub,
-    float4* xyoa_s, float4* bck_s, float4* col_s, int32_t* __restrict__ tile_work SC_DIAG_PARAM(dbg)) {
+    float4* xyoa_s, float4* bck_s, float4* col_s, int32_t* __restrict__ tile_work, int bucket_src SC_DIAG_PARAM(dbg)) {
     constexpr int B = SC_WALK_B;
     using Pixels = ScLanePixels<NSUB>;
     constexpr int NP = Pixels::NP, PPL = Pixels::PPL;
@@ -171,7 +171,20 @@
     const unsigned long long pc_begin = SC_DIAG_CLOCK(prof), pr_begin = SC_DIAG_REALTIME(prof);
     unsigned long long pc_stage = 0, pc_issue = 0, pc_blend = 0, pc_first = 0, pc_batches = 0, pc_splats = 0;
     int range_start, range_end;
-    sc_tile_range(isect_offsets, tflat, total_tiles, n_isects, range_start, range_end);
+    int bit = 0;
+    if (!TRACK && !PACKED && bucket_src) {
+        const int stw = (tile_width + 1) >> 1, sth = (tile_height + 1) >> 1;
+        const int sb = (cam * sth + (tile.tyi >> 1)) * stw + (tile.txi >> 1);
+        bit = 28 + (((tile.tyi & 1) << 1) | (tile.txi & 1));
+        const int s = isect_offsets[sb], e = isect_offsets[sb + 1];
+        range_start = min(max(s, 0), n_isects);
+        range_end = min(max(e, range_start), n_isects);
+    } else
+        sc_tile_range(isect_offsets, tflat, total_tiles, n_isects, range_start, range_end);
+    using Stage = ScStage<CDIM, PACKED>;
+    auto id_at = [&](int idx) -> int {
+        return bit ? Stage::bucket_id_at(flatten_ids, idx, range_end, N, bit) : Stage::id_at(flatten_ids, idx, range_end, N);
+    };
     const int num_batches = (range_end - range_start + B - 1) / B;
     int walked = 0;
     const ScRect rect = px.rect(tile, sub, width, height);
@@ -196,8 +209,8 @@
     const ScSplatArrays in = {means2d, conics, colors, opacities};
     ScStage<CDIM, PACKED> st;
     st.clear();
-    st.load(st.id_at(flatten_ids, range_start + lane, range_end, N), in);
-    st.g_next = st.id_at(flatten_ids, range_start + B + lane, range_end, N);
+    st.load(id_at(range_start + lane), in);
+    st.g_next = id_at(range_start + B + lane);
 
     for (int b = 0; b < num_batches; ++b) {
         if (all_done()) break;
@@ -209,7 +222,8 @@
         walked += 4;
         int bsz = sc_cull_compact<true>(st, rect, __int_as_float(batch_start + lane), 0.f, xyoa_s, bck_s, col_s);
         const unsigned long long pc1 = SC_DIAG_CLOCK(prof);
-        st.advance(in, flatten_ids, batch_start + 2 * B + lane, range_end, N);
+        st.load(st.g_next, in);
+        st.g_next = id_at(batch_start + 2 * B + lane);
         if (SC_DIAG_BIT(dbg, 1)) bsz = 0;
         const unsigned long long pc2 = SC_DIAG_CLOCK(prof);
         if (bsz > 0) {
@@ -315,7 +329,7 @@
     const int32_t* __restrict__ isect_offsets, const int32_t* __restrict__ flatten_ids, int n_isects,
     float* __restrict__ render_colors, float* __restrict__ render_alphas,
     int32_t* __restrict__ last_ids, int map_mode, const int32_t* __restrict__ order,
-    int32_t* __restrict__ tile_work SC_DIAG_PARAM(dbg)) {
+    int32_t* __restrict__ tile_work, int bucket_src SC_DIAG_PARAM(dbg)) {
     __shared__ float4 xyoa_s[SC_WALK_B + 1];
     __shared__ float4 bck_s[SC_WALK_B + 1];
     __shared__ float4 col_s[SC_WALK_B + 1];
@@ -339,13 +353,13 @@
     if (kind == 0)
         raster_item<CDIM, TRACK, 1, PACKED, ED, PLANAR>(means2d, conics, colors, opacities, backgrounds, tile_masks, N, width, height,
                                     tile_width, tile_height, total_tiles, isect_offsets, flatten_ids, n_isects,
-                                    render_colors, render_alphas, last_ids, tflat, 0, xyoa_s, bck_s, col_s, tile_work
-                                    SC_DIAG_ARG(dbg));
+                                    render_colors, render_alphas, last_ids, tflat, 0, xyoa_s, bck_s, col_s, tile_work,
+                                    bucket_src SC_DIAG_ARG(dbg));
     else
         raster_item<CDIM, TRACK, 2, PACKED, ED, PLANAR>(means2d, conics, colors, opacities, backgrounds, tile_masks, N, width, height,
                                     tile_width, tile_height, total_tiles, isect_offsets, flatten_ids, n_isects,
                                     render_colors, render_alphas, last_ids, tflat, kind - 1, xyoa_s, bck_s, col_s,
-                                    tile_work SC_DIAG_ARG(dbg));
+                                    tile_work, bucket_src SC_DIAG_ARG(dbg));
 }
 
 }
@@ -367,7 +381,7 @@
                               const int32_t* isect_offsets, const int32_t* flatten_ids,
                               int64_t n_isects, float* render_colors, float* render_alphas,
                               int32_t* last_ids, const int32_t* tile_order, int32_t* tile_work,
-                              sc_stream_t stream, int epilogue) {
+                              sc_stream_t stream, int epilogue, int bucket_src = 0) {
     if (C < 0 || N < 0 || D < 1 || D > SC_MAX_CDIM || width <= 0 || height <= 0) return SC_EINVAL;
     if (tile_size < 1 || tile_size > 32 || tile_width <= 0 || tile_height <= 0) return SC_EINVAL;
     if (n_isects < 0 || n_isects > 0x7fffffffLL) return SC_EINVAL;
@@ -387,6 +401,7 @@
     const bool ed = (epilogue & 1) != 0;
     const bool planar = (epilogue & 4) != 0;
     if (planar && (packed || ed || last_ids)) return SC_EUNSUPPORTED;
+    if (bucket_src && (packed || ed || last_ids || !(variant >= 3 && tile_size == 16 && (D == 3 || D == 4)))) return SC_EUNSUPPORTED;
     if (variant >= 3 && tile_size == 16 && (D == 3 || D == 4)) {
         if ((int64_t)C * tile_width * tile_height >= (1 << 29)) return SC_EINVAL;
         const int total_tiles = C * tile_width * tile_height;
@@ -396,7 +411,7 @@
     hipLaunchKernelGGL((raster_fwd_wave_kernel<CD, TR, PK, EDP, ##__VA_ARGS__>), dim3(n_blocks), dim3(64), 0, sc_s(stream), means2d, \
                        conics, colors, opacities, backgrounds, tile_masks, NS, width, height, tile_width,           \
                        tile_height, total_tiles, isect_offsets, flatten_ids, (int)n_isects, render_colors,         \
-                       render_alphas, last_ids, g_sc_raster_map, tile_order, tile_work SC_DIAG_ARG(g_sc_debug[1] & 0xff))
+                       render_alphas, last_ids, g_sc_raster_map, tile_order, tile_work, bucket_src SC_DIAG_ARG(g_sc_debug[1] & 0xff))
         if (planar) { if (D == 4) SC_LAUNCH_WAVE(4, false, false, false, true); else SC_LAUNCH_WAVE(3, false, false, false, true); }
         else if (packed) { if (ed) SC_LAUNCH_WAVE(4, false, true, true); else SC_LAUNCH_WAVE(4, false, true, false); }
         else if (D == 4) {
@@ -467,6 +482,20 @@
 }
 
 
+extern "C" int sc_rasterize_fwd_buckets(const float* means2d, const float* conics, const float* colors,
+                                        const float* opacities, const float* backgrounds,
+                                        const uint8_t* tile_masks, int C, int N, int D, int width, int height,
+                                        int tile_size, int tile_width, int tile_height,
+                                        const int32_t* super_offsets, const int32_t* super_ids,
+                                        int64_t n_records, float* render_colors, float* render_alphas,
+                                        const int32_t* tile_order, int32_t* tile_work, int planar, sc_stream_t stream) {
+    if (tile_size != 16) return SC_EUNSUPPORTED;
+    return rasterize_fwd_impl(means2d, conics, colors, opacities, backgrounds, tile_masks, C, N, D, width, height,
+                              tile_size, tile_width, tile_height, super_offsets, super_ids, n_records,
+                              render_colors, render_alphas, nullptr, tile_order, tile_work, stream, planar ? 4 : 0, 1);
+}
+
+
 extern "C" int sc_rasterize_fwd_packed(const float* records, const float* backgrounds, const uint8_t* tile_masks,
                                        int C, int N, int width, int height, int tile_width, int tile_height,
                                        const int32_t* isect_offsets, const int32_t* flatten_ids, int64_t n_isects,
diff --git a/street_crafter_amd/csrc/raster_walk.h b/street_crafter_amd/csrc/raster_walk.h
--- a/street_crafter_amd/csrc/raster_walk.h
+++ b/street_crafter_amd/csrc/raster_walk.h
@@ -87,6 +87,12 @@
     }
     static __device__ __forceinline__ int id_at(const int32_t* __restrict__ flatten_ids, int idx, int end, int n_splats) {
         return (idx < end) ? sc_safe_id(flatten_ids[idx], n_splats) : -1;
+    }
+    static __device__ __forceinline__ int bucket_id_at(const int32_t* __restrict__ super_ids, int idx, int end, int n_splats,
+                                                       int bit) {
+        if (idx >= end) return -1;
+        const unsigned e = (unsigned)super_ids[idx];
+        return ((e >> bit) & 1u) ? sc_safe_id((int)(e & 0x0fffffffu), n_splats) : -1;
     }
     template <class Extra = ScNoExtra>
     __device__ __forceinline__ void advance(const ScSplatArrays& in, const int32_t* __restrict__ flatten_ids, int idx2,
diff --git a/street_crafter_amd/isect.py b/street_crafter_amd/isect.py
--- a/street_crafter_amd/isect.py
+++ b/street_crafter_amd/isect.py
@@ -20,7 +20,8 @@
 
 
 class _Switches:
-    __slots__ = ("tile_order", "lazy_ids", "view_slots", "packed_records", "defer_isect", "planar_out", "fused_train")
+    __slots__ = ("tile_order", "lazy_ids", "view_slots", "packed_records", "defer_isect", "planar_out", "fused_train",
+                 "lazy_flatten")
 
     def __init__(self):
         self.tile_order = _env_on("SC_TILE_ORDER")
@@ -30,6 +31,7 @@
         self.defer_isect = _env_on("SC_DEFER_ISECT")
         self.planar_out = _env_on("SC_PLANAR_OUTPUT")
         self.fused_train = _env_on("SC_FUSED_TRAIN", False)
+        self.lazy_flatten = _env_on("SC_LAZY_FLATTEN")
 
     def flip(self, name: str, value: bool) -> bool:
         prev = getattr(self, name)
@@ -99,6 +101,10 @@
     return _SWITCH.flip("lazy_ids", enabled)
 
 
+def set_lazy_flatten_ids(enabled: bool) -> bool:
+    return _SWITCH.flip("lazy_flatten", enabled)
+
+
 def set_deferred_isect(enabled: bool) -> bool:
     return _SWITCH.flip("defer_isect", enabled)
 
@@ -143,11 +149,17 @@
         logging.getLogger("street_crafter_amd").warning(msg, *args)
 
 
-@torch.no_grad()
 def isect_tiles(means2d: Tensor, radii: Tensor, depths: Tensor, tile_size: int, tile_width: int,
                 tile_height: int, sort: bool = True, packed: bool = False,
                 n_cameras: Optional[int] = None, camera_ids: Optional[Tensor] = None,
                 gaussian_ids: Optional[Tensor] = None) -> Tuple[Tensor, Tensor, Tensor]:
+    training = torch.is_grad_enabled() and (means2d.requires_grad or depths.requires_grad)
+    with torch.no_grad():
+        return _isect_tiles(means2d, radii, depths, tile_size, tile_width, tile_height, sort, packed, n_cameras,
+                            not training)
+
+
+def _isect_tiles(means2d, radii, depths, tile_size, tile_width, tile_height, sort, packed, n_cameras, lazy_flat):
     if packed:
         raise NotImplementedError("packed=True is not supported (reference passes packed=False)")
     view_cams = getattr(means2d, "_sc_viewmats", None)
@@ -163,7 +175,7 @@
     mode = _ISECT_MODE["mode"] if sort else "radix"
     if mode == "bin":
         res = _isect_tiles_bin(means2d, radii, depths, C, N, tile_size, tile_width, tile_height, st,
-                               viewmats=view_cams, defer=True)
+                               viewmats=view_cams, defer=True, lazy_flat=lazy_flat)
         if res is not None:
             return res[:3]
     return _isect_tiles_radix(means2d, radii, depths, C, N, tile_size, tile_width, tile_height, sort, st)
@@ -283,14 +295,16 @@
 
 class _BinCall:
     __slots__ = ("b", "st", "dev", "inputs", "depths", "C", "N", "grid", "offsets", "meta_dev", "ws0", "slot", "seq",
-                 "eager_ids", "key", "pred", "ids", "fids", "flat", "n_isects", "ids_ref")
-
-    def __init__(self, b, st, inputs, C, N, grid, offsets, meta_dev, ws0, slot, eager_ids):
+                 "eager_ids", "key", "pred", "ids", "fids", "flat", "n_isects", "ids_ref", "buckets", "sids", "soffs",
+                 "n_records", "flat_filled", "flat_ref")
+
+    def __init__(self, b, st, inputs, C, N, grid, offsets, meta_dev, ws0, slot, eager_ids, buckets=False):
         self.b, self.st, self.dev = b, st, offsets.device
         self.inputs, self.depths, self.C, self.N, self.grid = inputs, inputs[2], C, N, grid
         self.offsets, self.meta_dev, self.ws0, self.slot, self.seq = offsets, meta_dev, ws0, slot, slot.seq
         self.eager_ids, self.key = eager_ids, (self.dev.index, C, N, *grid)
         self.pred = self.ids = self.fids = self.flat = self.n_isects = self.ids_ref = None
+        self.buckets, self.sids, self.soffs, self.n_records, self.flat_filled, self.flat_ref = buckets, None, None, 0, not buckets, None
 
     def read_meta(self):
         if self.b.wait_i64(self.slot.ptr + 32, self.seq, 2_000_000) != 0:
@@ -299,6 +313,11 @@
         return tuple(map(int, self.slot.view[:4]))
 
     def launch(self, capacities):
+        if self.buckets:
+            rc, self.sids, self.soffs = self.b.isect_bin_sort_buckets(
+                *self.inputs, *self.grid, self.meta_dev, self.ws0, int(capacities[0]), int(capacities[1]),
+                int(capacities[2]), self.st)
+            return rc
         rc, self.ids, self.fids = self.b.isect_bin_sort(
             *self.inputs, *self.grid, self.offsets, self.meta_dev, self.ws0, int(capacities[0]), int(capacities[1]),
             int(capacities[2]), bool(self.eager_ids), self.st)
@@ -326,16 +345,39 @@
             _lib.check(rc, "sc_isect_bin_sort")
         cap = _STATE.bucket_cap.get("v") or _STATE.bucket_cap.setdefault("v", int(_lib.load().sc_isect_bin_bucket_capacity()))
         _STATE.record(self.key, (n_isects, n_records, max_super), cap)
-        self.flat, self.n_isects = self.fids[:n_isects], n_isects
+        if self.buckets:
+            if n_isects == 0:
+                self.soffs.zero_()
+            self.flat, self.n_records = torch.empty(n_isects, dtype=torch.int32, device=self.dev), n_records
+        else:
+            self.flat = self.fids[:n_isects]
+        self.n_isects = n_isects
         self.inputs = self.meta_dev = self.ws0 = None
         return n_isects
 
-    def fill_ids(self, buf):
+    def _behind_sort(self, buf):
         cur = _stream(buf)
         if cur != self.st:
             ev = torch.cuda.Event()
             ev.record(torch.cuda.ExternalStream(self.st, device=self.dev))
             torch.cuda.current_stream(self.dev).wait_event(ev)
+        return cur
+
+    def ensure_flat(self, _buf=None):
+        if self.flat_filled:
+            return
+        if self.n_isects:
+            rc = self.b.isect_emit_tiles(self.sids, self.soffs, self.offsets, self.n_records, self.flat,
+                                         self._behind_sort(self.flat))
+            _lib.check(rc, "sc_isect_emit_tiles")
+        self.flat_filled = True
+        lazy = self.flat_ref() if self.flat_ref is not None else None
+        if lazy is not None:
+            lazy.__dict__["_sc_fill"] = None
+
+    def fill_ids(self, buf):
+        self.ensure_flat()
+        cur = self._behind_sort(buf)
         _lib.check(_lib.load().sc_isect_ids_rebuild(self.flat.data_ptr(), self.offsets.data_ptr(), self.depths.data_ptr(),
                                                     self.C, self.N, self.grid[1], self.grid[2], self.n_isects,
                                                     buf.data_ptr(), cur), "sc_isect_ids_rebuild")
@@ -348,12 +390,22 @@
 
     def deferred(self):
         pending = _PendingIsect(self.settle_deferred)
-        flatten_ids = _LazyTensor(self.fids[:0], None, pending.resolve)
+        if self.buckets:
+            flatten_ids = self.lazy_flat(pending.resolve)
+        else:
+            flatten_ids = _LazyTensor(self.fids[:0], None, pending.resolve)
         isect_ids = _LazyTensor(torch.empty(0, dtype=torch.int64, device=self.dev), self.fill_ids, pending.resolve)
         pending.flat_ref, pending.ids_ref = weakref.ref(flatten_ids), weakref.ref(isect_ids)
         self.slot.pending, self.ids_ref = weakref.ref(pending), pending.ids_ref
         self.file_offsets(isect_ids)
         return isect_ids, flatten_ids
+
+    def lazy_flat(self, resolve=None):
+        buf = self.flat if resolve is None else torch.empty(0, dtype=torch.int32, device=self.dev)
+        t = _LazyTensor(buf, self.ensure_flat, resolve)
+        t.__dict__["_sc_buckets"] = self
+        self.flat_ref = weakref.ref(t)
+        return t
 
     def settle_deferred(self):
         n_isects = self.settle()
@@ -361,6 +413,10 @@
             return self.flat, torch.empty(n_isects, dtype=torch.int64, device=self.dev), self.file_offsets
         with torch.cuda.stream(torch.cuda.ExternalStream(self.st, device=self.dev)):
             _, ids, flat = _isect_tiles_radix(*self.inputs, self.C, self.N, *self.grid, True, self.st)
+        self.flat_filled, self.sids, self.soffs = True, None, None
+        lazy = self.flat_ref() if self.flat_ref is not None else None
+        if lazy is not None:
+            lazy.__dict__["_sc_fill"] = None
         isect_ids = self.ids_ref()
         if isect_ids is not None:
             isect_ids.__dict__["_sc_fill"] = None
@@ -368,7 +424,7 @@
 
 
 def _isect_tiles_bin(means2d, radii, depths, C, N, tile_size, tile_width, tile_height, st, want_ids=True,
-                     viewmats=None, defer=False):
+                     viewmats=None, defer=False, lazy_flat=False):
     dev = means2d.device
     b = _lib.binding()
     slots = _PINNED_META.__dict__.setdefault("slots", {})
@@ -396,7 +452,8 @@
     if rc:
         _lib.check(rc, "sc_isect_bin_count")
     eager_ids = want_ids and not _SWITCH.lazy_ids
-    call = _BinCall(b, st, (means2d, radii, depths), C, N, grid, offsets, meta_dev, ws0, slot, eager_ids)
+    buckets = bool(lazy_flat) and want_ids and not eager_ids and _SWITCH.lazy_flatten and grid[0] == 16
+    call = _BinCall(b, st, (means2d, radii, depths), C, N, grid, offsets, meta_dev, ws0, slot, eager_ids, buckets)
     pred = _STATE.prediction.get(call.key)
     if pred is not None:
         rc = call.launch(pred)
@@ -414,7 +471,7 @@
         isect_ids = (call.ids[:n_isects] if eager_ids
                      else _LazyTensor(torch.empty(n_isects, dtype=torch.int64, device=dev), call.fill_ids))
         call.file_offsets(isect_ids)
-    return tiles_per_gauss, isect_ids, call.flat, offsets
+    return tiles_per_gauss, isect_ids, (call.lazy_flat() if buckets else call.flat), offsets
 
 
 @torch.no_grad()
diff --git a/street_crafter_amd/rendering.py b/street_crafter_amd/rendering.py
--- a/street_crafter_amd/rendering.py
+++ b/street_crafter_amd/rendering.py
@@ -11,7 +11,8 @@
 from .isect import (_ISECT_MODE, _PINNED_META, _RAW_STREAM, _STATE, _SWITCH, _BinCall, _MetaSlot,
                     _OperatorState, _PendingIsect, _Switches, _bin_launch_ran, _check_isect_count, _isect_tiles_bin,
                     _isect_tiles_radix, _p, _req, _stream, _tile_work, _view_registry, _warn_once, _ws,
-                    isect_offset_encode, isect_tiles, set_deferred_isect, set_isect_mode, set_lazy_isect_ids)
+                    isect_offset_encode, isect_tiles, set_deferred_isect, set_isect_mode, set_lazy_flatten_ids,
+                    set_lazy_isect_ids)
 
 __all__ = ["fully_fused_projection", "isect_tiles", "isect_offset_encode", "spherical_harmonics",
            "rasterize_to_pixels", "rasterization"]
@@ -296,7 +297,18 @@
                 st = side.cuda_stream
         rc = -3
         last_ids = None
-        if _SWITCH.planar_out and not needs_bwd and int(tile_size) == 16 and D in (3, 4):
+        planar = _SWITCH.planar_out and not needs_bwd and int(tile_size) == 16 and D in (3, 4)
+        if type(flatten_ids) is _BinCall:
+            call = flatten_ids
+            rc, render_colors, render_alphas = b.rasterize_fwd_buckets(
+                means2d, conics, colors, opacities, backgrounds, masks, int(width), int(height), int(tile_size), tw, th,
+                call.soffs, call.sids, call.n_records, order, work, bool(planar), st)
+            if rc not in (0, -3):
+                _lib.check(rc, "sc_rasterize_fwd_buckets")
+            if rc == -3:
+                call.ensure_flat()
+                flatten_ids = call.flat
+        if rc == -3 and planar:
             rc, render_colors, render_alphas = b.rasterize_fwd_planar(
                 means2d, conics, colors, opacities, backgrounds, masks, int(width), int(height), int(tile_size),
                 isect_offsets, flatten_ids, order, work, st)
@@ -346,6 +358,17 @@
         return (v_means2d, v_conics, v_colors, v_opacities, v_bg, None, None, None, None, None, None, None, None)
 
 
+def _buckets_of(flatten_ids, isect_offsets, tile_size, colors, needs_grad):
+    call = flatten_ids.__dict__.get("_sc_buckets")
+    if (call is None or needs_grad or not _SWITCH.lazy_flatten or not flatten_ids.untouched or int(tile_size) != 16
+            or colors.shape[-1] not in (3, 4) or call.offsets is not isect_offsets):
+        return None
+    flatten_ids.resolve_shape()
+    if call.sids is None or call.flat_filled:
+        return None
+    return call
+
+
 class _AbsgradTarget:
     __slots__ = ("tensor",)
 
@@ -366,9 +389,14 @@
     colors = _req(colors, "colors")
     opacities = _req(opacities, "opacities")
     isect_offsets = _req(isect_offsets, "isect_offsets", torch.int32)
+    buckets = None
     if type(flatten_ids) is _LazyTensor:
-        flatten_ids = flatten_ids.plain()
-    flatten_ids = _req(flatten_ids, "flatten_ids", torch.int32)
+        buckets = _buckets_of(flatten_ids, isect_offsets, tile_size, colors,
+                              _needs_grad(means2d_c, conics, colors, opacities, backgrounds))
+        if buckets is None:
+            flatten_ids = flatten_ids.plain()
+    if buckets is None:
+        flatten_ids = _req(flatten_ids, "flatten_ids", torch.int32)
     C, N = opacities.shape
     D = colors.shape[-1]
     assert means2d_c.shape == (C, N, 2), means2d_c.shape
@@ -396,8 +424,8 @@
                                       int(image_height), int(tile_size), isect_offsets, flatten_ids, bool(absgrad), order,
                                       work, caller_means2d, _RAW_STREAM)
     return _call(_Rasterize, means2d_c, conics, colors, opacities, backgrounds, masks, int(image_width),
-                            int(image_height), int(tile_size), isect_offsets, flatten_ids, bool(absgrad),
-                            _AbsgradTarget(caller_means2d))
+                            int(image_height), int(tile_size), isect_offsets, flatten_ids if buckets is None else buckets,
+                            bool(absgrad), _AbsgradTarget(caller_means2d))
 
 
 def camera_centers(viewmats: Tensor) -> Tensor:
```

After: 3105. -2.2%, worse.
